# pathwaycom/pathway

Measured on AMD Instinct MI355X. Metric: events/sec (whole node) on WordCount stream + p50 RAG query latency at fixed QPS, higher is better.
Workload: dtype int64/string-dict; 1 GPU; model=wordcount: stream -> groupby(word).count -> output deltas, global_batch=4000000, seq_len=1, parallelism=dp1 (shard exchange: RCCL all-to-all), vocab=50000, ingest=bytes, emitted_delta_rows=126750000, dict_misses=0

## Files before the change

pathway_amd/ops/__init__.py:

```python

from __future__ import annotations

import contextlib
import ctypes
import os
from typing import Sequence

import torch

_THIS = os.path.dirname(os.path.abspath(__file__))
_LIB_PATH = os.path.join(_THIS, "libpwhip.so")

_lib = None
_load_error: Exception | None = None


def _try_load():
    global _lib, _load_error
    if _lib is not None:
        return _lib
    try:
        if not os.path.exists(_LIB_PATH):
            from pathway_amd.ops import build as _build

            _build.build(verbose=False)
        _lib = ctypes.CDLL(_LIB_PATH)
        _lib.pw_hash128_words.restype = ctypes.c_int
        _lib.pw_value_hash.restype = ctypes.c_int
        _lib.pw_varlen_hash.restype = ctypes.c_int
        _lib.pw_run_starts.restype = ctypes.c_int
    except Exception as e:
        _load_error = e
        _lib = None
    return _lib


def lib_available() -> bool:
    return _try_load() is not None


def require_lib():
    lib = _try_load()
    if lib is None:
        raise RuntimeError(
            f"pathway_amd native HIP library missing on a GPU host: {_load_error}"
        )
    return lib


def _stream_ptr() -> ctypes.c_void_p:
    return ctypes.c_void_p(torch.cuda.current_stream().cuda_stream)


def hash128_words_gpu(words: Sequence[torch.Tensor]) -> tuple[torch.Tensor, torch.Tensor]:
    lib = require_lib()
    n = words[0].shape[0]
    lo = torch.empty(n, dtype=torch.int64, device=words[0].device)
    hi = torch.empty(n, dtype=torch.int64, device=words[0].device)
    arr = (ctypes.c_void_p * len(words))(
        *[ctypes.c_void_p(w.contiguous().data_ptr()) for w in words]
    )
    rc = lib.pw_hash128_words(
        arr,
        ctypes.c_int(len(words)),
        ctypes.c_int64(n),
        ctypes.c_void_p(lo.data_ptr()),
        ctypes.c_void_p(hi.data_ptr()),
        _stream_ptr(),
    )
    if rc != 0:
        raise RuntimeError(f"pw_hash128_words failed: hip error {rc}")
    return lo, hi


def value_hash_gpu(payload: torch.Tensor, tag: int) -> tuple[torch.Tensor, torch.Tensor]:
    lib = require_lib()
    payload = payload.contiguous()
    n = payload.shape[0]
    lo = torch.empty(n, dtype=torch.int64, device=payload.device)
    hi = torch.empty(n, dtype=torch.int64, device=payload.device)
    rc = lib.pw_value_hash(
        ctypes.c_void_p(payload.data_ptr()),
        ctypes.c_uint64(tag),
        ctypes.c_int64(n),
        ctypes.c_void_p(lo.data_ptr()),
        ctypes.c_void_p(hi.data_ptr()),
        _stream_ptr(),
    )
    if rc != 0:
        raise RuntimeError(f"pw_value_hash failed: hip error {rc}")
    return lo, hi


def varlen_hash_gpu(
    bytes_t: torch.Tensor, offsets: torch.Tensor, tag: int
) -> tuple[torch.Tensor, torch.Tensor]:
    lib = require_lib()
    n = offsets.shape[0] - 1
    lo = torch.empty(n, dtype=torch.int64, device=bytes_t.device)
    hi = torch.empty(n, dtype=torch.int64, device=bytes_t.device)
    rc = lib.pw_varlen_hash(
        ctypes.c_void_p(bytes_t.contiguous().data_ptr()),
        ctypes.c_void_p(offsets.contiguous().data_ptr()),
        ctypes.c_uint64(tag),
        ctypes.c_int64(n),
        ctypes.c_void_p(lo.data_ptr()),
        ctypes.c_void_p(hi.data_ptr()),
        _stream_ptr(),
    )
    if rc != 0:
        raise RuntimeError(f"pw_varlen_hash failed: hip error {rc}")
    return lo, hi


def run_starts_gpu(words: Sequence[torch.Tensor]) -> torch.Tensor:
    lib = require_lib()
    n = words[0].shape[0]
    starts = torch.empty(n, dtype=torch.bool, device=words[0].device)
    arr = (ctypes.c_void_p * len(words))(
        *[ctypes.c_void_p(w.contiguous().data_ptr()) for w in words]
    )
    rc = lib.pw_run_starts(
        arr,
        ctypes.c_int(len(words)),
        ctypes.c_int64(n),
        ctypes.c_void_p(starts.data_ptr()),
        _stream_ptr(),
    )
    if rc != 0:
        raise RuntimeError(f"pw_run_starts failed: hip error {rc}")
    return starts


def host_hash128_bytes(data: bytes) -> tuple[int, int]:
    lib = require_lib()
    lo = ctypes.c_uint64()
    hi = ctypes.c_uint64()
    lib.pw_host_hash128_bytes(data, ctypes.c_int64(len(data)), ctypes.byref(lo), ctypes.byref(hi))
    return lo.value, hi.value


def _ptr_arr(tensors):
    return (ctypes.c_void_p * len(tensors))(
        *[ctypes.c_void_p(t.data_ptr()) for t in tensors]
    )


def searchsorted_gpu(
    sorted_words: Sequence[torch.Tensor],
    query_words: Sequence[torch.Tensor],
    side: str = "left",
) -> torch.Tensor:
    lib = require_lib()
    m = sorted_words[0].shape[0]
    nq = query_words[0].shape[0]
    out = torch.empty(nq, dtype=torch.int64, device=query_words[0].device)
    s = [t.contiguous() for t in sorted_words]
    q = [t.contiguous() for t in query_words]
    rc = lib.pw_searchsorted(
        _ptr_arr(s),
        _ptr_arr(q),
        ctypes.c_int(len(s)),
        ctypes.c_int64(m),
        ctypes.c_int64(nq),
        ctypes.c_int(1 if side == "right" else 0),
        ctypes.c_void_p(out.data_ptr()),
        _stream_ptr(),
    )
    if rc != 0:
        raise RuntimeError(f"pw_searchsorted failed: hip error {rc}")
    return out


def lookup_gpu(
    sorted_words: Sequence[torch.Tensor], query_words: Sequence[torch.Tensor]
) -> tuple[torch.Tensor, torch.Tensor]:
    lib = require_lib()
    m = sorted_words[0].shape[0]
    nq = query_words[0].shape[0]
    pos = torch.empty(nq, dtype=torch.int64, device=query_words[0].device)
    found = torch.empty(nq, dtype=torch.bool, device=query_words[0].device)
    s = [t.contiguous() for t in sorted_words]
    q = [t.contiguous() for t in query_words]
    rc = lib.pw_lookup(
        _ptr_arr(s),
        _ptr_arr(q),
        ctypes.c_int(len(s)),
        ctypes.c_int64(m),
        ctypes.c_int64(nq),
        ctypes.c_void_p(pos.data_ptr()),
        ctypes.c_void_p(found.data_ptr()),
        _stream_ptr(),
    )
    if rc != 0:
        raise RuntimeError(f"pw_lookup failed: hip error {rc}")
    return pos, found


def key_range_gpu(
    sorted_words: Sequence[torch.Tensor], query_words: Sequence[torch.Tensor]
) -> tuple[torch.Tensor, torch.Tensor]:
    lib = require_lib()
    m = sorted_words[0].shape[0]
    nq = query_words[0].shape[0]
    lo = torch.empty(nq, dtype=torch.int64, device=query_words[0].device)
    hi = torch.empty(nq, dtype=torch.int64, device=query_words[0].device)
    s = [t.contiguous() for t in sorted_words]
    q = [t.contiguous() for t in query_words]
    rc = lib.pw_key_range(
        _ptr_arr(s),
        _ptr_arr(q),
        ctypes.c_int(len(s)),
        ctypes.c_int64(m),
        ctypes.c_int64(nq),
        ctypes.c_void_p(lo.data_ptr()),
        ctypes.c_void_p(hi.data_ptr()),
        _stream_ptr(),
    )
    if rc != 0:
        raise RuntimeError(f"pw_key_range failed: hip error {rc}")
    return lo, hi


SEG_FIRST = 0
SEG_MIN = 1
SEG_MAX = 2
SEG_SELECT_LONG = 4096
SEG_DISTINCT_CAPACITY = 4096
SEG_DISTINCT_MAX_PASSES = 64

multiset_path_counts = {"select": 0, "distinct": 0, "host": 0, "torch": 0}


def _check_ranges(lo: torch.Tensor, hi: torch.Tensor, weights: torch.Tensor):
    for name, t in (("lo", lo), ("hi", hi), ("weights", weights)):
        if t.dtype != torch.int64 or t.dim() != 1 or not t.is_contiguous():
            raise ValueError(f"{name} must be a contiguous 1-D int64 tensor")
        if not t.is_cuda or t.device != weights.device:
            raise ValueError(f"{name} must be on the weights' GPU")
    if lo.shape[0] != hi.shape[0]:
        raise ValueError("lo and hi differ in length")


def seg_select_gpu(
    lo: torch.Tensor,
    hi: torch.Tensor,
    weights: torch.Tensor,
    key: torch.Tensor | None,
    mode: int,
    long_rows: int | None = None,
) -> torch.Tensor:
    lib = require_lib()
    _check_ranges(lo, hi, weights)
    m = weights.shape[0]
    if mode == SEG_FIRST:
        if key is not None:
            raise ValueError("SEG_FIRST reads no key")
        kind, kptr = 0, None
    elif mode in (SEG_MIN, SEG_MAX):
        if key is None:
            raise ValueError("SEG_MIN / SEG_MAX need a key column")
        if key.dtype == torch.int64:
            kind = 1
        elif key.dtype == torch.float64:
            kind = 2
        else:
            raise ValueError(f"key must be int64 or float64, not {key.dtype}")
        if key.shape != (m,) or not key.is_contiguous() or key.device != weights.device:
            raise ValueError("key must be a contiguous 1-D column of the store")
        kptr = key.data_ptr()
    else:
        raise ValueError(f"unknown mode {mode}")
    long_rows = SEG_SELECT_LONG if long_rows is None else int(long_rows)
    if long_rows < 64:
        raise ValueError("long_rows must be at least 64")
    nq = lo.shape[0]
    sel = torch.empty(nq, dtype=torch.int64, device=weights.device)
    rc = lib.pw_seg_select(
        ctypes.c_void_p(lo.data_ptr()),
        ctypes.c_void_p(hi.data_ptr()),
        ctypes.c_int64(nq),
        ctypes.c_void_p(weights.data_ptr()),
        ctypes.c_void_p(kptr),
        ctypes.c_int(kind),
        ctypes.c_int64(m),
        ctypes.c_int(mode),
        ctypes.c_int64(long_rows),
        ctypes.c_void_p(sel.data_ptr()),
        _stream_ptr(),
    )
    if rc != 0:
        raise RuntimeError(f"pw_seg_select failed: error {rc}")
    return sel


def seg_distinct_gpu(
    lo: torch.Tensor,
    hi: torch.Tensor,
    weights: torch.Tensor,
    values: torch.Tensor,
    table_capacity: int | None = None,
) -> tuple[torch.Tensor, torch.Tensor, torch.Tensor]:
    lib = require_lib()
    _check_ranges(lo, hi, weights)
    m = weights.shape[0]
    if (
        values.dtype != torch.int64
        or values.shape != (m,)
        or not values.is_contiguous()
        or values.device != weights.device
    ):
        raise ValueError("values must be a contiguous 1-D int64 column of the store")
    cap = SEG_DISTINCT_CAPACITY if table_capacity is None else int(table_capacity)
    if cap < 64 or cap > 8192 or cap & (cap - 1):
        raise ValueError("table_capacity must be a power of two in [64, 8192]")
    nq = lo.shape[0]
    dev = weights.device
    count = torch.empty(nq, dtype=torch.int64, device=dev)
    first = torch.empty(nq, dtype=torch.int64, device=dev)
    status = torch.empty(nq, dtype=torch.int32, device=dev)
    rc = lib.pw_seg_distinct(
        ctypes.c_void_p(lo.data_ptr()),
        ctypes.c_void_p(hi.data_ptr()),
        ctypes.c_int64(nq),
        ctypes.c_void_p(weights.data_ptr()),
        ctypes.c_void_p(values.data_ptr()),
        ctypes.c_int64(m),
        ctypes.c_int64(cap),
        ctypes.c_int64(int(GC_BUCKET_MAX_LOAD * cap)),
        ctypes.c_int64(GC_BUCKET_MAX_PROBE),
        ctypes.c_void_p(count.data_ptr()),
        ctypes.c_void_p(first.data_ptr()),
        ctypes.c_void_p(status.data_ptr()),
        _stream_ptr(),
    )
    if rc != 0:
        raise RuntimeError(f"pw_seg_distinct failed: error {rc}")
    return count, first, status


def pool_hash_gpu(
    codes: torch.Tensor,
    pool_lo: torch.Tensor,
    pool_hi: torch.Tensor,
    none_lo: int,
    none_hi: int,
) -> tuple[torch.Tensor, torch.Tensor]:
    lib = require_lib()
    n = codes.shape[0]
    lo = torch.empty(n, dtype=torch.int64, device=codes.device)
    hi = torch.empty(n, dtype=torch.int64, device=codes.device)
    rc = lib.pw_pool_hash(
        ctypes.c_void_p(codes.contiguous().data_ptr()),
        ctypes.c_void_p(pool_lo.contiguous().data_ptr()),
        ctypes.c_void_p(pool_hi.contiguous().data_ptr()),
        ctypes.c_uint64(none_lo & ((1 << 64) - 1)),
        ctypes.c_uint64(none_hi & ((1 << 64) - 1)),
        ctypes.c_int64(n),
        ctypes.c_void_p(lo.data_ptr()),
        ctypes.c_void_p(hi.data_ptr()),
        _stream_ptr(),
    )
    if rc != 0:
        raise RuntimeError(f"pw_pool_hash failed: hip error {rc}")
    return lo, hi


def varlen_hash_se_gpu(
    bytes_t: torch.Tensor,
    starts: torch.Tensor,
    ends: torch.Tensor,
    tag: int,
) -> tuple[torch.Tensor, torch.Tensor]:
    lib = require_lib()
    n = starts.shape[0]
    lo = torch.empty(n, dtype=torch.int64, device=bytes_t.device)
    hi = torch.empty(n, dtype=torch.int64, device=bytes_t.device)
    rc = lib.pw_varlen_hash_se(
        ctypes.c_void_p(bytes_t.contiguous().data_ptr()),
        ctypes.c_void_p(starts.contiguous().data_ptr()),
        ctypes.c_void_p(ends.contiguous().data_ptr()),
        ctypes.c_uint64(tag),
        ctypes.c_int64(n),
        ctypes.c_void_p(lo.data_ptr()),
        ctypes.c_void_p(hi.data_ptr()),
        _stream_ptr(),
    )
    if rc != 0:
        raise RuntimeError(f"pw_varlen_hash_se failed: hip error {rc}")
    return lo, hi


def hash_agg_gpu(
    k0: torch.Tensor,
    k1: torch.Tensor,
    contribs: Sequence[torch.Tensor],
    expected_uniques: int | None = None,
) -> tuple[torch.Tensor, torch.Tensor, list, torch.Tensor] | None:
    lib = require_lib()
    n = k0.shape[0]
    dev = k0.device
    nacc = len(contribs)
    est = n if expected_uniques is None else min(max(expected_uniques, 512), n)
    cap = 1 << max(10, (2 * est - 1).bit_length())
    out_cap = min(n, cap)
    tk0 = torch.empty(cap, dtype=torch.int64, device=dev)
    tk1 = torch.zeros(cap, dtype=torch.int64, device=dev)
    rep = torch.zeros(cap, dtype=torch.int64, device=dev)
    taccs = [torch.zeros(cap, dtype=torch.int64, device=dev) for _ in range(nacc)]
    counter = torch.zeros(2, dtype=torch.int32, device=dev)
    out_k0 = torch.empty(out_cap, dtype=torch.int64, device=dev)
    out_k1 = torch.empty(out_cap, dtype=torch.int64, device=dev)
    out_rep = torch.empty(out_cap, dtype=torch.int64, device=dev)
    out_accs = [
        torch.empty(out_cap, dtype=torch.int64, device=dev) for _ in range(nacc)
    ]
    carr = (ctypes.c_void_p * max(nacc, 1))(
        *[ctypes.c_void_p(c.contiguous().data_ptr()) for c in contribs]
    )
    tarr = (ctypes.c_void_p * max(nacc, 1))(
        *[ctypes.c_void_p(c.data_ptr()) for c in taccs]
    )
    oarr = (ctypes.c_void_p * max(nacc, 1))(
        *[ctypes.c_void_p(c.data_ptr()) for c in out_accs]
    )
    rc = lib.pw_hash_agg(
        ctypes.c_void_p(k0.contiguous().data_ptr()),
        ctypes.c_void_p(k1.contiguous().data_ptr()),
        carr,
        ctypes.c_int(nacc),
        ctypes.c_int64(n),
        ctypes.c_void_p(tk0.data_ptr()),
        ctypes.c_void_p(tk1.data_ptr()),
        tarr,
        ctypes.c_void_p(rep.data_ptr()),
        ctypes.c_int64(cap),
        ctypes.c_void_p(counter.data_ptr()),
        ctypes.c_void_p(out_k0.data_ptr()),
        ctypes.c_void_p(out_k1.data_ptr()),
        oarr,
        ctypes.c_void_p(out_rep.data_ptr()),
        ctypes.c_void_p(counter.data_ptr() + 4),
        _stream_ptr(),
    )
    if rc != 0:
        raise RuntimeError(f"pw_hash_agg failed: hip error {rc}")
    m, overflowed = (int(x) for x in counter.tolist())
    if overflowed:
        return None
    return (
        out_k0.narrow(0, 0, m),
        out_k1.narrow(0, 0, m),
        [a.narrow(0, 0, m) for a in out_accs],
        out_rep.narrow(0, 0, m),
    )


def seg_reduce_words_gpu(
    words: Sequence[torch.Tensor], contribs: Sequence[torch.Tensor]
) -> tuple[list, torch.Tensor, list]:
    lib = require_lib()
    n = words[0].shape[0]
    dev = words[0].device
    nw = len(words)
    nacc = len(contribs)
    words = [w.contiguous() for w in words]
    nblocks = (n + 255) // 256
    block_counts = torch.empty(nblocks, dtype=torch.int32, device=dev)
    warr = (ctypes.c_void_p * nw)(
        *[ctypes.c_void_p(w.data_ptr()) for w in words]
    )
    rc = lib.pw_seg_reduce_count(
        warr,
        ctypes.c_int(nw),
        ctypes.c_int64(n),
        ctypes.c_void_p(block_counts.data_ptr()),
        ctypes.c_int64(nblocks),
        _stream_ptr(),
    )
    if rc != 0:
        raise RuntimeError(f"pw_seg_reduce_count failed: hip error {rc}")
    csum = torch.cumsum(block_counts.to(torch.int64), 0)
    nseg = int(csum[-1].item())
    bases = torch.cat(
        [torch.zeros(1, dtype=torch.int64, device=dev), csum[:-1]]
    )
    out_words = [torch.empty(nseg, dtype=torch.int64, device=dev) for _ in range(nw)]
    out_first = torch.empty(nseg, dtype=torch.int64, device=dev)
    out_accs = [torch.zeros(nseg, dtype=torch.int64, device=dev) for _ in range(nacc)]
    carr = (ctypes.c_void_p * max(nacc, 1))(
        *[ctypes.c_void_p(c.contiguous().data_ptr()) for c in contribs]
    )
    oarr = (ctypes.c_void_p * max(nacc, 1))(
        *[ctypes.c_void_p(c.data_ptr()) for c in out_accs]
    )
    owarr = (ctypes.c_void_p * nw)(
        *[ctypes.c_void_p(w.data_ptr()) for w in out_words]
    )
    rc = lib.pw_seg_reduce_emit(
        warr,
        ctypes.c_int(nw),
        carr,
        ctypes.c_int(nacc),
        ctypes.c_int64(n),
        ctypes.c_void_p(bases.data_ptr()),
        owarr,
        ctypes.c_void_p(out_first.data_ptr()),
        oarr,
        ctypes.c_int64(nblocks),
        _stream_ptr(),
    )
    if rc != 0:
        raise RuntimeError(f"pw_seg_reduce_emit failed: hip error {rc}")
    return out_words, out_first, out_accs


def seg_reduce_gpu(
    k0: torch.Tensor, k1: torch.Tensor, contribs: Sequence[torch.Tensor]
) -> tuple[torch.Tensor, torch.Tensor, torch.Tensor, list]:
    out_words, out_first, out_accs = seg_reduce_words_gpu([k0, k1], contribs)
    return out_words[0], out_words[1], out_first, out_accs


_gc_temp_bytes: dict[int, int] = {}
_gc_temp_bytes_prefix: dict[int, int] = {}

_PW_GC_FULL_SORT = bool(os.environ.get("PW_GC_FULL_SORT"))

class _GcPathCounts(dict):

    bucket = 0

    def __getitem__(self, key):
        return self.bucket if key == "bucket" else dict.__getitem__(self, key)

    def __setitem__(self, key, value):
        if key == "bucket":
            self.bucket = value
        else:
            dict.__setitem__(self, key, value)


gc_path_counts = _GcPathCounts({"prefix": 0, "fallback": 0, "full": 0})

_PW_NO_GC_PARTITION = bool(os.environ.get("PW_NO_GC_PARTITION"))
_PW_GC_PART_DIRECT = bool(os.environ.get("PW_GC_PART_DIRECT"))
gc_bucket_layout_counts = {"partition": 0, "gather": 0}
GC_PART_TILE = 8192
GC_PART_MAX_BITS = 8

_gc_bucket_scope = False


@contextlib.contextmanager
def gc_bucket_scope(on: bool):
    global _gc_bucket_scope
    old, _gc_bucket_scope = _gc_bucket_scope, bool(on)
    try:
        yield
    finally:
        _gc_bucket_scope = old

gc_last_dirty_runs = 0

GC_BUCKET_MAX_LOAD = 0.5
GC_BUCKET_BITS = 8
GC_BUCKET_ROWS_FACTOR = 4
GC_BUCKET_MAX_PROBE = 128
GC_BUCKET_ROWS_FLOOR = 65536

_gc_bucket_caps: dict[int, int] = {}


def gc_bucket_capacity_limit(nacc: int) -> int:
    cap = _gc_bucket_caps.get(nacc)
    if cap is None:
        fn = require_lib().pw_gc_bucket_max_capacity
        fn.restype = ctypes.c_int64
        cap = int(fn(ctypes.c_int(nacc)))
        if cap < 2:
            raise RuntimeError("pw_gc_bucket_max_capacity failed")
        _gc_bucket_caps[nacc] = cap
    return cap


def gc_bucket_capacity(nacc: int) -> int:
    return min(gc_bucket_capacity_limit(nacc), 2048)


def gc_bucket_key_budget(nacc: int, bucket_bits: int = GC_BUCKET_BITS,
                         table_capacity: int | None = None) -> int:
    cap = table_capacity or gc_bucket_capacity(nacc)
    return (1 << bucket_bits) * int(GC_BUCKET_MAX_LOAD * cap)


def _gc_temp(lib, n: int, prefix: bool, dev) -> tuple[torch.Tensor, int]:
    cache = _gc_temp_bytes_prefix if prefix else _gc_temp_bytes
    tbytes = cache.get(n)
    if tbytes is None:
        fn = lib.pw_gc_temp_bytes_prefix if prefix else lib.pw_gc_temp_bytes
        fn.restype = ctypes.c_int64
        tbytes = int(fn(ctypes.c_int64(n)))
        if tbytes <= 0:
            raise RuntimeError("pw_gc_temp_bytes failed")
        cache[n] = tbytes
    return torch.empty(tbytes, dtype=torch.uint8, device=dev), tbytes


def _group_combine_two_sorts(keys_n2, contribs):
    k0, k1 = keys_n2[:, 0], keys_n2[:, 1]
    perm = torch.argsort(k1, stable=True)
    perm = perm.index_select(0, torch.argsort(k0.index_select(0, perm), stable=True))
    uk0, uk1, first_sorted, accs = seg_reduce_gpu(
        k0.index_select(0, perm),
        k1.index_select(0, perm),
        [c.index_select(0, perm) for c in contribs],
    )
    return uk0, uk1, perm.index_select(0, first_sorted), accs


def _gc_part_hist_entries(lib, n: int, bucket_bits: int) -> int:
    fn = lib.pw_gc_part_hist_entries
    fn.restype = ctypes.c_int64
    entries = int(fn(ctypes.c_int64(n), ctypes.c_int(bucket_bits)))
    if entries <= 0:
        raise RuntimeError("pw_gc_part_hist_entries failed")
    tile = lib.pw_gc_part_tile
    tile.restype = ctypes.c_int64
    assert int(tile()) == GC_PART_TILE
    return entries


def _gc_aligned_keys(keys_n2: torch.Tensor) -> torch.Tensor:
    return keys_n2.clone() if keys_n2.data_ptr() % 16 else keys_n2


def gc_partition_gpu(
    keys_n2: torch.Tensor, contribs: Sequence[torch.Tensor], bucket_bits: int
) -> tuple[torch.Tensor, torch.Tensor, torch.Tensor, list]:
    lib = require_lib()
    n = keys_n2.shape[0]
    dev = keys_n2.device
    nacc = len(contribs)
    assert keys_n2.dim() == 2 and keys_n2.shape[1] == 2
    assert keys_n2.dtype == torch.int64
    assert 2 <= n < 2**32 - 1 and nacc <= 8 and 1 <= bucket_bits <= 8
    if keys_n2.stride() != (2, 1):
        keys_n2 = keys_n2.contiguous()
    keys_n2 = _gc_aligned_keys(keys_n2)
    contribs = [c.contiguous() for c in contribs]
    assert all(c.dtype == torch.int64 and c.shape == (n,) for c in contribs)
    nb = 1 << bucket_bits
    hist = _gc_part_hist_entries(lib, n, bucket_bits)
    part64 = torch.empty((2 + nacc, n), dtype=torch.int64, device=dev)
    scratch32 = torch.empty(hist + n + nb + 1, dtype=torch.int32, device=dev)
    ctl = torch.empty(2, dtype=torch.int64, device=dev)
    carr = (ctypes.c_void_p * max(nacc, 1))(
        *[ctypes.c_void_p(c.data_ptr()) for c in contribs]
    )
    parr = (ctypes.c_void_p * max(nacc, 1))(
        *[ctypes.c_void_p(part64[2 + a].data_ptr()) for a in range(nacc)]
    )
    rc = lib.pw_gc_partition(
        ctypes.c_void_p(keys_n2.data_ptr()),
        ctypes.c_int64(n),
        ctypes.c_int(bucket_bits),
        carr,
        ctypes.c_int(nacc),
        ctypes.c_void_p(scratch32.data_ptr()),
        ctypes.c_void_p(part64.data_ptr()),
        ctypes.c_void_p(scratch32[hist:].data_ptr()),
        parr,
        ctypes.c_void_p(scratch32[hist + n :].data_ptr()),
        ctypes.c_void_p(ctl.data_ptr()),
        ctypes.c_int(int(_PW_GC_PART_DIRECT)),
        _stream_ptr(),
    )
    if rc != 0:
        raise RuntimeError(f"pw_gc_partition failed: hip error {rc}")
    u32 = lambda t: t.to(torch.int64) & 0xFFFFFFFF
    return (
        u32(scratch32[hist + n :]),
# ... 637 lines not shown
    )
    if rc != 0:
        raise RuntimeError(f"pw_merge_consolidate_emit failed: {rc}")
    return out_words, out_accs, rep


def group_update_gpu(
    a_words: Sequence[torch.Tensor],
    a_accs: Sequence[torch.Tensor],
    b_words: Sequence[torch.Tensor],
    b_accs: Sequence[torch.Tensor],
    out_slots: Sequence[int],
):
    lib = require_lib()
    m = a_words[0].shape[0]
    n = b_words[0].shape[0]
    nacc = len(a_accs)
    assert len(a_words) == 2 and len(b_words) == 2
    assert len(b_accs) == nacc and 1 <= nacc <= 8
    slots = sorted(set(int(s) for s in out_slots))
    assert all(0 <= s < nacc for s in slots)
    mask = 0
    for s in slots:
        mask |= 1 << s
    device = b_words[0].device
    nthreads = max(1, (m + n + 7) // 8)
    counts = torch.empty(nthreads * 4, dtype=torch.int32, device=device)
    bases = torch.empty(nthreads * 3, dtype=torch.int64, device=device)
    totals = torch.empty(3, dtype=torch.int64, device=device)
    wA = [t.contiguous() for t in a_words]
    wB = [t.contiguous() for t in b_words]
    aA = [t.contiguous() for t in a_accs]
    aB = [t.contiguous() for t in b_accs]
    for t in wA + wB + aA + aB:
        assert t.dtype == torch.int64
    rc = lib.pw_group_update_count(
        _ptr_arr(wA),
        _ptr_arr(aA),
        _ptr_arr(wB),
        _ptr_arr(aB),
        ctypes.c_int(nacc),
        ctypes.c_uint(mask),
        ctypes.c_int64(m),
        ctypes.c_int64(n),
        ctypes.c_void_p(counts.data_ptr()),
        ctypes.c_void_p(bases.data_ptr()),
        ctypes.c_void_p(totals.data_ptr()),
        ctypes.c_int64(nthreads),
        _stream_ptr(),
    )
    if rc != 0:
        raise RuntimeError(f"pw_group_update_count failed: {rc}")
    n_keep, n_ret, n_ins = totals.tolist()
    n_out = n_ret + n_ins

    def i64(k):
        return torch.empty(k, dtype=torch.int64, device=device)

    out_words = [i64(n_keep) for _ in range(2)]
    out_accs = [i64(n_keep) for _ in range(nacc)]
    rep = i64(n_keep)
    keys = torch.empty((n_out, 2), dtype=torch.int64, device=device)
    diffs = i64(n_out)
    vals = {s: i64(n_out) for s in slots}
    src = i64(n_out)
    varr = (ctypes.c_void_p * 8)(
        *[ctypes.c_void_p(vals[s].data_ptr() if s in vals else 0) for s in range(8)]
    )
    rc = lib.pw_group_update_emit(
        _ptr_arr(wA),
        _ptr_arr(aA),
        _ptr_arr(wB),
        _ptr_arr(aB),
        ctypes.c_int(nacc),
        ctypes.c_uint(mask),
        ctypes.c_int64(m),
        ctypes.c_int64(n),
        ctypes.c_void_p(bases.data_ptr()),
        ctypes.c_int64(n_ret),
        ctypes.c_int64(nthreads),
        _ptr_arr(out_words),
        _ptr_arr(out_accs),
        ctypes.c_void_p(rep.data_ptr()),
        ctypes.c_void_p(keys.data_ptr()),
        ctypes.c_void_p(diffs.data_ptr()),
        varr,
        ctypes.c_void_p(src.data_ptr()),
        _stream_ptr(),
    )
    if rc != 0:
        raise RuntimeError(f"pw_group_update_emit failed: {rc}")
    return out_words, out_accs, rep, keys, diffs, [vals[s] for s in slots], src


def radix_sort64_gpu(keys: torch.Tensor) -> tuple[torch.Tensor, torch.Tensor]:
    lib = require_lib()
    n = keys.shape[0]
    device = keys.device
    perm = torch.arange(n, dtype=torch.int64, device=device)
    if n <= 1:
        return keys.clone(), perm
    nblocks = max(1, min(1024, (n + (64 * 64) - 1) // (64 * 64)))
    chunk = (n + nblocks * 64 - 1) // (nblocks * 64)
    ka = torch.empty(n, dtype=torch.int64, device=device)
    kb = torch.empty(n, dtype=torch.int64, device=device)
    pa = perm
    pb = torch.empty(n, dtype=torch.int64, device=device)
    rc = lib.pw_radix_flip(
        ctypes.c_void_p(keys.contiguous().data_ptr()),
        ctypes.c_void_p(ka.data_ptr()),
        ctypes.c_int64(n),
        _stream_ptr(),
    )
    if rc != 0:
        raise RuntimeError(f"pw_radix_flip failed: {rc}")
    counts = torch.empty(256 * nblocks, dtype=torch.int32, device=device)
    for p in range(8):
        shift = p * 8
        rc = lib.pw_radix_count(
            ctypes.c_void_p(ka.data_ptr()),
            ctypes.c_int64(n),
            ctypes.c_int(shift),
            ctypes.c_int64(nblocks),
            ctypes.c_int64(chunk),
            ctypes.c_void_p(counts.data_ptr()),
            _stream_ptr(),
        )
        if rc != 0:
            raise RuntimeError(f"pw_radix_count failed: {rc}")
        csum = torch.cumsum(counts.to(torch.int64), 0)
        bases = torch.zeros_like(csum)
        bases[1:] = csum[:-1]
        rc = lib.pw_radix_scatter(
            ctypes.c_void_p(ka.data_ptr()),
            ctypes.c_void_p(pa.data_ptr()),
            ctypes.c_int64(n),
            ctypes.c_int(shift),
            ctypes.c_int64(nblocks),
            ctypes.c_int64(chunk),
            ctypes.c_void_p(bases.data_ptr()),
            ctypes.c_void_p(kb.data_ptr()),
            ctypes.c_void_p(pb.data_ptr()),
            _stream_ptr(),
        )
        if rc != 0:
            raise RuntimeError(f"pw_radix_scatter failed: {rc}")
        ka, kb = kb, ka
        pa, pb = pb, pa
    out = torch.empty(n, dtype=torch.int64, device=device)
    rc = lib.pw_radix_unflip(
        ctypes.c_void_p(ka.data_ptr()),
        ctypes.c_void_p(out.data_ptr()),
        ctypes.c_int64(n),
        _stream_ptr(),
    )
    if rc != 0:
        raise RuntimeError(f"pw_radix_unflip failed: {rc}")
    return out, pa


def scan_positions_gpu(buf: torch.Tensor, target: int) -> torch.Tensor:
    lib = require_lib()
    n = buf.shape[0]
    device = buf.device
    nblocks = max(1, min(2048, (n + 4095) // 4096))
    counts = torch.empty(nblocks, dtype=torch.int64, device=device)
    rc = lib.pw_scan_positions(
        ctypes.c_void_p(buf.contiguous().data_ptr()),
        ctypes.c_int64(n),
        ctypes.c_int(int(target)),
        ctypes.c_void_p(counts.data_ptr()),
        ctypes.c_int64(nblocks),
        _stream_ptr(),
    )
    if rc != 0:
        raise RuntimeError(f"pw_scan_positions failed: {rc}")
    csum = torch.cumsum(counts, 0)
    total = int(csum[-1].item())
    bases = torch.zeros(nblocks, dtype=torch.int64, device=device)
    bases[1:] = csum[:-1]
    out = torch.empty(total, dtype=torch.int64, device=device)
    rc = lib.pw_scan_emit(
        ctypes.c_void_p(buf.contiguous().data_ptr()),
        ctypes.c_int64(n),
        ctypes.c_int(int(target)),
        ctypes.c_void_p(bases.data_ptr()),
        ctypes.c_int64(nblocks),
        ctypes.c_void_p(out.data_ptr()),
        _stream_ptr(),
    )
    if rc != 0:
        raise RuntimeError(f"pw_scan_emit failed: {rc}")
    return out


def sort_repair_gpu(
    k0_sorted: torch.Tensor,
    k1_sorted: torch.Tensor,
    perm: torch.Tensor,
    passes: int = 4,
) -> None:
    lib = require_lib()
    n = k0_sorted.shape[0]
    if n < 2:
        return
    rc = lib.pw_sort_repair(
        ctypes.c_void_p(k0_sorted.data_ptr()),
        ctypes.c_void_p(k1_sorted.data_ptr()),
        ctypes.c_void_p(perm.data_ptr()),
        ctypes.c_int64(n),
        ctypes.c_int(int(passes)),
        _stream_ptr(),
    )
    if rc != 0:
        raise RuntimeError(f"pw_sort_repair failed: hip error {rc}")


def gather_cols_gpu(idx: torch.Tensor, cols: list) -> list:
    lib = require_lib()
    m = idx.shape[0]
    outs: list = [None] * len(cols)
    fused_pos: list[int] = []
    for i, c in enumerate(cols):
        if c.dim() == 1 and c.element_size() == 8 and c.is_contiguous():
            fused_pos.append(i)
        else:
            outs[i] = c[idx] if c.dim() > 1 else c.index_select(0, idx)
    idx = idx.contiguous()
    for start in range(0, len(fused_pos), 8):
        group = fused_pos[start : start + 8]
        srcs = (ctypes.c_void_p * len(group))()
        dsts = (ctypes.c_void_p * len(group))()
        for k, i in enumerate(group):
            c = cols[i]
            out = torch.empty(m, dtype=c.dtype, device=c.device)
            outs[i] = out
            srcs[k] = c.data_ptr()
            dsts[k] = out.data_ptr()
        rc = lib.pw_gather_cols(
            ctypes.c_void_p(idx.data_ptr()),
            ctypes.c_int64(m),
            ctypes.c_int(len(group)),
            srcs,
            dsts,
            _stream_ptr(),
        )
        if rc != 0:
            raise RuntimeError(f"pw_gather_cols failed: {rc}")
    return outs


def intern_error_message(e: int) -> str:
    parts = []
    if e & 1:
        parts.append("probe bound hit (table full)")
    if e & 2:
        parts.append("slot, claimer row or span out of range")
    if e & 4:
        parts.append("dictionary arrays or byte arena too small")
    return "device dictionary intern failed: " + "; ".join(parts or [str(e)])


def gather_spans_gpu(
    buf: torch.Tensor,
    starts: torch.Tensor,
    ends: torch.Tensor,
    first_rows: torch.Tensor,
    n_new: torch.Tensor,
    base: torch.Tensor,
    arena: torch.Tensor,
    cursor: torch.Tensor,
    tok_off: torch.Tensor,
    tok_len: torch.Tensor,
    err: torch.Tensor,
) -> None:
    lib = require_lib()
    nrows = starts.shape[0]
    if nrows == 0:
        return
    for t in (buf, starts, ends, first_rows, arena, tok_off, tok_len):
        assert t.is_contiguous()
    rc = lib.pw_gather_spans(
        ctypes.c_void_p(buf.data_ptr()),
        ctypes.c_int64(buf.shape[0]),
        ctypes.c_void_p(starts.data_ptr()),
        ctypes.c_void_p(ends.data_ptr()),
        ctypes.c_int64(nrows),
        ctypes.c_void_p(first_rows.data_ptr()),
        ctypes.c_void_p(n_new.data_ptr()),
        ctypes.c_void_p(base.data_ptr()),
        ctypes.c_void_p(arena.data_ptr()),
        ctypes.c_int64(arena.shape[0]),
        ctypes.c_void_p(cursor.data_ptr()),
        ctypes.c_void_p(tok_off.data_ptr()),
        ctypes.c_void_p(tok_len.data_ptr()),
        ctypes.c_int64(min(tok_off.shape[0], tok_len.shape[0])),
        ctypes.c_void_p(err.data_ptr()),
        _stream_ptr(),
    )
    if rc != 0:
        raise RuntimeError(f"pw_gather_spans failed: hip error {rc}")


class DeviceHashTable:

    def __init__(self, klo: torch.Tensor, khi: torch.Tensor,
                 vals: torch.Tensor | None = None, reserve: int = 0):
        require_lib()
        m = klo.shape[0]
        device = klo.device
        self.nslots = self.slots_for(max(m, int(reserve)))
        self.err = torch.zeros(1, dtype=torch.int64, device=device)
        self._alloc(device)
        self.insert(klo, khi, vals)

    @staticmethod
    def slots_for(m: int) -> int:
        return 1 << max(4, (2 * m - 1).bit_length()) if m else 16

    def _alloc(self, device) -> None:
        nslots = self.nslots
        self.tab_lo = torch.empty(nslots, dtype=torch.int64, device=device)
        self.tab_hi = torch.empty(nslots, dtype=torch.int64, device=device)
        self.tab_val = torch.full((nslots,), -1, dtype=torch.int64, device=device)

    def insert(self, klo: torch.Tensor, khi: torch.Tensor,
               vals: torch.Tensor | None = None) -> None:
        lib = require_lib()
        m = klo.shape[0]
        if not m:
            return
        klo, khi = klo.contiguous(), khi.contiguous()
        vals = vals.contiguous() if vals is not None else None
        rc = lib.pw_ht_build(
            ctypes.c_void_p(klo.data_ptr()),
            ctypes.c_void_p(khi.data_ptr()),
            ctypes.c_void_p(vals.data_ptr()) if vals is not None else None,
            ctypes.c_int64(m),
            ctypes.c_void_p(self.tab_lo.data_ptr()),
            ctypes.c_void_p(self.tab_hi.data_ptr()),
            ctypes.c_void_p(self.tab_val.data_ptr()),
            ctypes.c_int64(self.nslots),
            _stream_ptr(),
        )
        if rc != 0:
            raise RuntimeError(f"pw_ht_build failed: hip error {rc}")

    def fits(self, size: int) -> bool:
        return 2 * int(size) <= self.nslots

    def rebuild(self, size: int, klo: torch.Tensor, khi: torch.Tensor) -> None:
        self.nslots = self.slots_for(max(int(size), klo.shape[0]))
        self._alloc(klo.device)
        self.insert(klo, khi, None)

    def intern(
        self,
        qlo: torch.Tensor,
        qhi: torch.Tensor,
        base,
        pool_lo: torch.Tensor,
        pool_hi: torch.Tensor,
        front: "DeviceHashTable | None" = None,
    ) -> tuple[torch.Tensor, torch.Tensor, torch.Tensor]:
        lib = require_lib()
        n = qlo.shape[0]
        device = qlo.device
        codes = torch.empty(n, dtype=torch.int64, device=device)
        first_rows = torch.empty(n, dtype=torch.int64, device=device)
        if n == 0:
            return codes, first_rows, torch.zeros(1, dtype=torch.int64, device=device)
        if not torch.is_tensor(base):
            base = torch.tensor([int(base)], dtype=torch.int64, device=device)
        assert base.dtype == torch.int64 and base.is_contiguous()
        assert pool_lo.is_contiguous() and pool_hi.is_contiguous()
        qlo, qhi = qlo.contiguous(), qhi.contiguous()
        nblocks = max(1, min(2048, (n + 4095) // 4096))
        work = torch.empty(nblocks + 1, dtype=torch.int64, device=device)
        pend = torch.empty(n, dtype=torch.uint8, device=device)
        n_new = work[nblocks:]
        rc = lib.pw_ht_intern(
            ctypes.c_void_p(qlo.data_ptr()),
            ctypes.c_void_p(qhi.data_ptr()),
            ctypes.c_int64(n),
            ctypes.c_void_p(self.tab_lo.data_ptr()),
            ctypes.c_void_p(self.tab_hi.data_ptr()),
            ctypes.c_void_p(self.tab_val.data_ptr()),
            ctypes.c_int64(self.nslots),
            ctypes.c_void_p(front.tab_lo.data_ptr() if front else None),
            ctypes.c_void_p(front.tab_hi.data_ptr() if front else None),
            ctypes.c_void_p(front.tab_val.data_ptr() if front else None),
            ctypes.c_int64(front.nslots if front else 0),
            ctypes.c_void_p(base.data_ptr()),
            ctypes.c_void_p(pool_lo.data_ptr()),
            ctypes.c_void_p(pool_hi.data_ptr()),
            ctypes.c_int64(min(pool_lo.shape[0], pool_hi.shape[0])),
            ctypes.c_void_p(codes.data_ptr()),
            ctypes.c_void_p(pend.data_ptr()),
            ctypes.c_void_p(first_rows.data_ptr()),
            ctypes.c_void_p(work.data_ptr()),
            ctypes.c_int64(nblocks),
            ctypes.c_void_p(n_new.data_ptr()),
            ctypes.c_void_p(self.err.data_ptr()),
            _stream_ptr(),
        )
        if rc != 0:
            raise RuntimeError(f"pw_ht_intern failed: hip error {rc}")
        return codes, first_rows, n_new

    def check_error(self) -> None:
        e = int(self.err.item())
        if e:
            raise RuntimeError(intern_error_message(e))

    def probe(self, qlo: torch.Tensor, qhi: torch.Tensor) -> tuple[torch.Tensor, torch.Tensor]:
        lib = require_lib()
        nq = qlo.shape[0]
        out = torch.empty(nq, dtype=torch.int64, device=qlo.device)
        found = torch.empty(nq, dtype=torch.bool, device=qlo.device)
        if nq == 0:
            return out, found
        rc = lib.pw_ht_probe(
            ctypes.c_void_p(qlo.contiguous().data_ptr()),
            ctypes.c_void_p(qhi.contiguous().data_ptr()),
            ctypes.c_int64(nq),
            ctypes.c_void_p(self.tab_lo.data_ptr()),
            ctypes.c_void_p(self.tab_hi.data_ptr()),
            ctypes.c_void_p(self.tab_val.data_ptr()),
            ctypes.c_int64(self.nslots),
            ctypes.c_void_p(out.data_ptr()),
            ctypes.c_void_p(found.data_ptr()),
            _stream_ptr(),
        )
        if rc != 0:
            raise RuntimeError(f"pw_ht_probe failed: hip error {rc}")
        return out, found


def gather_all(idx: torch.Tensor, tensors: list) -> list:
    if tensors and tensors[0].is_cuda and idx.shape[0] > 2048 and lib_available():
        return gather_cols_gpu(idx, list(tensors))
    return [
        t.index_select(0, idx) if t.dim() == 1 else t[idx] for t in tensors
    ]
```

pathway_amd/ops/csrc/hip/pw_kernels.hip:

```cpp
#include <hip/hip_runtime.h>
#include <stdint.h>
#include <stdio.h>

#include <cstring>
#include <rocprim/rocprim.hpp>

#include "../xxhash_common.h"

#define PW_BLOCK 256
#define PW_MAX_GRID 2048

static inline int pw_grid(int64_t n) {
  int64_t g = (n + PW_BLOCK - 1) / PW_BLOCK;
  if (g > PW_MAX_GRID) g = PW_MAX_GRID;
  if (g < 1) g = 1;
  return (int)g;
}


struct WordPtrs {
  const uint64_t* p[20];
};

template <int W>
__global__ void k_hash128_words(WordPtrs ptrs, int64_t n, uint64_t* lo,
                                uint64_t* hi) {
  for (int64_t i = (int64_t)blockIdx.x * blockDim.x + threadIdx.x; i < n;
       i += (int64_t)gridDim.x * blockDim.x) {
    uint64_t w[W];
#pragma unroll
    for (int j = 0; j < W; ++j) w[j] = ptrs.p[j][i];
    lo[i] = pw_xxh64_words<W>(w, PW_SEED_LO);
    hi[i] = pw_xxh64_words<W>(w, PW_SEED_HI);
  }
}

extern "C" int pw_hash128_words(const void** word_ptrs, int nwords, int64_t n,
                                void* lo, void* hi, void* stream) {
  WordPtrs ptrs;
  for (int j = 0; j < nwords && j < 20; ++j)
    ptrs.p[j] = (const uint64_t*)word_ptrs[j];
  hipStream_t s = (hipStream_t)stream;
  dim3 grid(pw_grid(n)), block(PW_BLOCK);
#define CASE(W)                                                        \
  case W:                                                              \
    hipLaunchKernelGGL((k_hash128_words<W>), grid, block, 0, s, ptrs,  \
                       n, (uint64_t*)lo, (uint64_t*)hi);               \
    break;
  switch (nwords) {
    CASE(1) CASE(2) CASE(3) CASE(4) CASE(5) CASE(6) CASE(7) CASE(8)
    CASE(9) CASE(10) CASE(11) CASE(12) CASE(13) CASE(14) CASE(15) CASE(16)
    CASE(17) CASE(18) CASE(19) CASE(20)
    default:
      return -1;
  }
#undef CASE
  return (int)hipGetLastError();
}

__global__ void k_value_hash(const uint64_t* payload, uint64_t tag, int64_t n,
                             uint64_t* lo, uint64_t* hi) {
  for (int64_t i = (int64_t)blockIdx.x * blockDim.x + threadIdx.x; i < n;
       i += (int64_t)gridDim.x * blockDim.x) {
    uint64_t w[2] = {tag, payload[i]};
    lo[i] = pw_xxh64_words<2>(w, PW_SEED_LO);
    hi[i] = pw_xxh64_words<2>(w, PW_SEED_HI);
  }
}

extern "C" int pw_value_hash(const void* payload, uint64_t tag, int64_t n,
                             void* lo, void* hi, void* stream) {
  hipLaunchKernelGGL(k_value_hash, dim3(pw_grid(n)), dim3(PW_BLOCK), 0,
                     (hipStream_t)stream, (const uint64_t*)payload, tag, n,
                     (uint64_t*)lo, (uint64_t*)hi);
  return (int)hipGetLastError();
}

__device__ uint64_t pw_xxh64_long(const uint8_t* data, int64_t n, uint64_t tag,
                                  uint64_t seed);

__global__ void k_varlen_hash(const uint8_t* bytes, const int64_t* offsets,
                              uint64_t tag, int64_t n, uint64_t* lo,
                              uint64_t* hi) {
  for (int64_t i = (int64_t)blockIdx.x * blockDim.x + threadIdx.x; i < n;
       i += (int64_t)gridDim.x * blockDim.x) {
    int64_t a = offsets[i], b = offsets[i + 1];
    uint8_t buf[64];
    int64_t len = b - a;
    if (len <= 56) {
      uint64_t t = tag;
      __builtin_memcpy(buf, &t, 8);
      for (int64_t k = 0; k < len; ++k) buf[8 + k] = bytes[a + k];
      lo[i] = pw_xxh64_bytes(buf, 8 + len, PW_SEED_LO);
      hi[i] = pw_xxh64_bytes(buf, 8 + len, PW_SEED_HI);
    } else {
      lo[i] = pw_xxh64_long(bytes + a, len, tag, PW_SEED_LO);
      hi[i] = pw_xxh64_long(bytes + a, len, tag, PW_SEED_HI);
    }
  }
}

__device__ uint64_t pw_xxh64_long(const uint8_t* data, int64_t n, uint64_t tag,
                                  uint64_t seed) {
  uint64_t v1 = seed + PW_P1 + PW_P2;
  uint64_t v2 = seed + PW_P2;
  uint64_t v3 = seed;
  uint64_t v4 = seed - PW_P1;
  uint64_t a = tag, b, c, d;
  __builtin_memcpy(&b, data, 8);
  __builtin_memcpy(&c, data + 8, 8);
  __builtin_memcpy(&d, data + 16, 8);
  v1 = pw_round(v1, a);
  v2 = pw_round(v2, b);
  v3 = pw_round(v3, c);
  v4 = pw_round(v4, d);
  int64_t i = 24;
  while (i + 32 <= n) {
    __builtin_memcpy(&a, data + i, 8);
    __builtin_memcpy(&b, data + i + 8, 8);
    __builtin_memcpy(&c, data + i + 16, 8);
    __builtin_memcpy(&d, data + i + 24, 8);
    v1 = pw_round(v1, a);
    v2 = pw_round(v2, b);
    v3 = pw_round(v3, c);
    v4 = pw_round(v4, d);
    i += 32;
  }
  uint64_t h = pw_rotl64(v1, 1) + pw_rotl64(v2, 7) + pw_rotl64(v3, 12) +
               pw_rotl64(v4, 18);
  h = pw_merge_round(h, v1);
  h = pw_merge_round(h, v2);
  h = pw_merge_round(h, v3);
  h = pw_merge_round(h, v4);
  h += (uint64_t)(n + 8);
  while (i + 8 <= n) {
    uint64_t k;
    __builtin_memcpy(&k, data + i, 8);
    h ^= pw_round(0, k);
    h = pw_rotl64(h, 27) * PW_P1 + PW_P4;
    i += 8;
  }
  while (i + 4 <= n) {
    uint32_t k;
    __builtin_memcpy(&k, data + i, 4);
    h ^= (uint64_t)k * PW_P1;
    h = pw_rotl64(h, 23) * PW_P2 + PW_P3;
    i += 4;
  }
  while (i < n) {
    h ^= (uint64_t)data[i] * PW_P5;
    h = pw_rotl64(h, 11) * PW_P1;
    i += 1;
  }
  return pw_avalanche(h);
}

extern "C" int pw_varlen_hash(const void* bytes, const void* offsets,
                              uint64_t tag, int64_t n, void* lo, void* hi,
                              void* stream) {
  hipLaunchKernelGGL(k_varlen_hash, dim3(pw_grid(n)), dim3(PW_BLOCK), 0,
                     (hipStream_t)stream, (const uint8_t*)bytes,
                     (const int64_t*)offsets, tag, n, (uint64_t*)lo,
                     (uint64_t*)hi);
  return (int)hipGetLastError();
}


struct Words4 {
  const uint64_t* p[4];
};

__global__ void k_run_starts(Words4 w, int nw, int64_t n, bool* starts) {
  for (int64_t i = (int64_t)blockIdx.x * blockDim.x + threadIdx.x; i < n;
       i += (int64_t)gridDim.x * blockDim.x) {
    bool ne = (i == 0);
    if (i > 0) {
      for (int j = 0; j < nw; ++j) ne |= (w.p[j][i] != w.p[j][i - 1]);
    }
    starts[i] = ne;
  }
}

extern "C" int pw_run_starts(const void** word_ptrs, int nwords, int64_t n,
                             void* starts, void* stream) {
  Words4 w;
  for (int j = 0; j < nwords && j < 4; ++j) w.p[j] = (const uint64_t*)word_ptrs[j];
  hipLaunchKernelGGL(k_run_starts, dim3(pw_grid(n)), dim3(PW_BLOCK), 0,
                     (hipStream_t)stream, w, nwords, n, (bool*)starts);
  return (int)hipGetLastError();
}


extern "C" void pw_host_hash128_bytes(const void* data, int64_t n,
                                      uint64_t* lo, uint64_t* hi) {
  *lo = pw_xxh64_bytes((const uint8_t*)data, n, PW_SEED_LO);
  *hi = pw_xxh64_bytes((const uint8_t*)data, n, PW_SEED_HI);
}

extern "C" void pw_host_varlen_hash(const void* bytes, const int64_t* offsets,
                                    uint64_t tag, int64_t n, uint64_t* lo,
                                    uint64_t* hi) {
  const uint8_t* b = (const uint8_t*)bytes;
  for (int64_t i = 0; i < n; ++i) {
    int64_t a = offsets[i], e = offsets[i + 1];
    int64_t len = e - a;
    uint8_t stackbuf[4096];
    uint8_t* buf = stackbuf;
    if (len + 8 > (int64_t)sizeof(stackbuf)) buf = new uint8_t[len + 8];
    uint64_t t = tag;
    __builtin_memcpy(buf, &t, 8);
    __builtin_memcpy(buf + 8, b + a, len);
    lo[i] = pw_xxh64_bytes(buf, len + 8, PW_SEED_LO);
    hi[i] = pw_xxh64_bytes(buf, len + 8, PW_SEED_HI);
    if (buf != stackbuf) delete[] buf;
  }
}


struct SWords {
  const uint64_t* s[4];
  const uint64_t* q[4];
};

__device__ __forceinline__ int pw_cmp_row(const SWords& w, int nw, int64_t si,
                                          int64_t qi) {
  for (int j = 0; j < nw; ++j) {
    int64_t a = (int64_t)w.s[j][si];
    int64_t b = (int64_t)w.q[j][qi];
    if (a < b) return -1;
    if (a > b) return 1;
  }
  return 0;
}

template <bool RIGHT>
__global__ void k_searchsorted(SWords w, int nw, int64_t m, int64_t nq,
                               int64_t* out) {
  for (int64_t i = (int64_t)blockIdx.x * blockDim.x + threadIdx.x; i < nq;
       i += (int64_t)gridDim.x * blockDim.x) {
    int64_t lo = 0, hi = m;
    while (lo < hi) {
      int64_t mid = (lo + hi) >> 1;
      int c = pw_cmp_row(w, nw, mid, i);
      bool go_right = RIGHT ? (c <= 0) : (c < 0);
      if (go_right)
        lo = mid + 1;
      else
        hi = mid;
    }
    out[i] = lo;
  }
}

extern "C" int pw_searchsorted(const void** sorted_ptrs, const void** query_ptrs,
                               int nwords, int64_t m, int64_t nq, int right,
                               void* out, void* stream) {
  SWords w;
  for (int j = 0; j < nwords && j < 4; ++j) {
    w.s[j] = (const uint64_t*)sorted_ptrs[j];
    w.q[j] = (const uint64_t*)query_ptrs[j];
  }
  dim3 grid(pw_grid(nq)), block(PW_BLOCK);
  if (right)
    hipLaunchKernelGGL((k_searchsorted<true>), grid, block, 0,
                       (hipStream_t)stream, w, nwords, m, nq, (int64_t*)out);
  else
    hipLaunchKernelGGL((k_searchsorted<false>), grid, block, 0,
                       (hipStream_t)stream, w, nwords, m, nq, (int64_t*)out);
  return (int)hipGetLastError();
}

__global__ void k_lookup(SWords w, int nw, int64_t m, int64_t nq, int64_t* pos,
                         bool* found) {
  for (int64_t i = (int64_t)blockIdx.x * blockDim.x + threadIdx.x; i < nq;
       i += (int64_t)gridDim.x * blockDim.x) {
    int64_t lo = 0, hi = m;
    while (lo < hi) {
      int64_t mid = (lo + hi) >> 1;
      if (pw_cmp_row(w, nw, mid, i) < 0)
        lo = mid + 1;
      else
        hi = mid;
    }
    bool f = false;
    int64_t p = lo;
    if (lo < m && pw_cmp_row(w, nw, lo, i) == 0) f = true;
    if (p >= m) p = m > 0 ? m - 1 : 0;
    pos[i] = p;
    found[i] = f;
  }
}

extern "C" int pw_lookup(const void** sorted_ptrs, const void** query_ptrs,
                         int nwords, int64_t m, int64_t nq, void* pos,
                         void* found, void* stream) {
  SWords w;
  for (int j = 0; j < nwords && j < 4; ++j) {
    w.s[j] = (const uint64_t*)sorted_ptrs[j];
    w.q[j] = (const uint64_t*)query_ptrs[j];
  }
  hipLaunchKernelGGL(k_lookup, dim3(pw_grid(nq)), dim3(PW_BLOCK), 0,
                     (hipStream_t)stream, w, nwords, m, nq, (int64_t*)pos,
                     (bool*)found);
  return (int)hipGetLastError();
}

__global__ void k_key_range(SWords w, int nw, int64_t m, int64_t nq,
                            int64_t* lo_out, int64_t* hi_out) {
  for (int64_t i = (int64_t)blockIdx.x * blockDim.x + threadIdx.x; i < nq;
       i += (int64_t)gridDim.x * blockDim.x) {
    int64_t lo = 0, hi = m;
    while (lo < hi) {
      int64_t mid = (lo + hi) >> 1;
      if (pw_cmp_row(w, nw, mid, i) < 0)
        lo = mid + 1;
      else
        hi = mid;
    }
    int64_t left = lo;
    lo = left;
    hi = m;
    while (lo < hi) {
      int64_t mid = (lo + hi) >> 1;
      if (pw_cmp_row(w, nw, mid, i) <= 0)
        lo = mid + 1;
      else
        hi = mid;
    }
    lo_out[i] = left;
    hi_out[i] = lo;
  }
}

extern "C" int pw_key_range(const void** sorted_ptrs, const void** query_ptrs,
                            int nwords, int64_t m, int64_t nq, void* lo,
                            void* hi, void* stream) {
  SWords w;
  for (int j = 0; j < nwords && j < 4; ++j) {
    w.s[j] = (const uint64_t*)sorted_ptrs[j];
    w.q[j] = (const uint64_t*)query_ptrs[j];
  }
  hipLaunchKernelGGL(k_key_range, dim3(pw_grid(nq)), dim3(PW_BLOCK), 0,
                     (hipStream_t)stream, w, nwords, m, nq, (int64_t*)lo,
                     (int64_t*)hi);
  return (int)hipGetLastError();
}


__global__ void k_pool_hash(const int64_t* codes, const uint64_t* pool_lo,
                            const uint64_t* pool_hi, uint64_t none_lo,
                            uint64_t none_hi, int64_t n, uint64_t* lo,
                            uint64_t* hi) {
  for (int64_t i = (int64_t)blockIdx.x * blockDim.x + threadIdx.x; i < n;
       i += (int64_t)gridDim.x * blockDim.x) {
    int64_t c = codes[i];
    if (c >= 0) {
      lo[i] = pool_lo[c];
      hi[i] = pool_hi[c];
    } else {
      lo[i] = none_lo;
      hi[i] = none_hi;
    }
  }
}

extern "C" int pw_pool_hash(const void* codes, const void* pool_lo,
                            const void* pool_hi, uint64_t none_lo,
                            uint64_t none_hi, int64_t n, void* lo, void* hi,
                            void* stream) {
  hipLaunchKernelGGL(k_pool_hash, dim3(pw_grid(n)), dim3(PW_BLOCK), 0,
                     (hipStream_t)stream, (const int64_t*)codes,
                     (const uint64_t*)pool_lo, (const uint64_t*)pool_hi,
                     none_lo, none_hi, n, (uint64_t*)lo, (uint64_t*)hi);
  return (int)hipGetLastError();
}

__global__ void k_varlen_hash_se(const uint8_t* bytes, const int64_t* starts,
                                 const int64_t* ends, uint64_t tag, int64_t n,
                                 uint64_t* lo, uint64_t* hi) {
  for (int64_t i = (int64_t)blockIdx.x * blockDim.x + threadIdx.x; i < n;
       i += (int64_t)gridDim.x * blockDim.x) {
    int64_t a = starts[i], b = ends[i];
    uint8_t buf[64];
    int64_t len = b - a;
    if (len <= 56) {
      uint64_t t = tag;
      __builtin_memcpy(buf, &t, 8);
      for (int64_t k = 0; k < len; ++k) buf[8 + k] = bytes[a + k];
      lo[i] = pw_xxh64_bytes(buf, 8 + len, PW_SEED_LO);
      hi[i] = pw_xxh64_bytes(buf, 8 + len, PW_SEED_HI);
    } else {
      lo[i] = pw_xxh64_long(bytes + a, len, tag, PW_SEED_LO);
      hi[i] = pw_xxh64_long(bytes + a, len, tag, PW_SEED_HI);
    }
  }
}

extern "C" int pw_varlen_hash_se(const void* bytes, const void* starts,
                                 const void* ends, uint64_t tag, int64_t n,
                                 void* lo, void* hi, void* stream) {
  hipLaunchKernelGGL(k_varlen_hash_se, dim3(pw_grid(n)), dim3(PW_BLOCK), 0,
                     (hipStream_t)stream, (const uint8_t*)bytes,
                     (const int64_t*)starts, (const int64_t*)ends, tag, n,
                     (uint64_t*)lo, (uint64_t*)hi);
  return (int)hipGetLastError();
}


#define PW_HA_EMPTY 0x8000000000000000ULL

struct AccPtrs {
  const long long* p[8];
};
struct AccPtrsMut {
  long long* p[8];
};

__global__ void k_hash_agg(const long long* k0, const long long* k1,
                           AccPtrs contribs, int nacc, int64_t n,
                           unsigned long long* tk0, long long* tk1,
                           AccPtrsMut taccs, long long* rep, uint64_t mask,
                           unsigned int* overflow) {
  for (int64_t i = (int64_t)blockIdx.x * blockDim.x + threadIdx.x; i < n;
       i += (int64_t)gridDim.x * blockDim.x) {
    unsigned long long key0 = (unsigned long long)k0[i];
    long long key1 = k1[i];
    uint64_t slot = ((uint64_t)key0) & mask;
    for (uint64_t tries = 0; tries < 512 && tries <= mask; ++tries) {
      unsigned long long cur = tk0[slot];
      if (cur == PW_HA_EMPTY)
        cur = atomicCAS(&tk0[slot], PW_HA_EMPTY, key0);
      if (cur == PW_HA_EMPTY) {
        tk1[slot] = key1;
        rep[slot] = (long long)i;
        __threadfence();
      } else if (cur != key0) {
        slot = (slot + 1) & mask;
        continue;
      } else if (tk1[slot] != key1) {
        slot = (slot + 1) & mask;
        continue;
      }
      for (int a = 0; a < nacc; ++a)
        atomicAdd((unsigned long long*)&taccs.p[a][slot],
                  (unsigned long long)contribs.p[a][i]);
      goto next_row;
    }
    atomicOr(overflow, 1u);
  next_row:;
  }
}

__global__ void k_hash_agg_init(unsigned long long* tk0, uint64_t cap) {
  for (uint64_t i = (uint64_t)blockIdx.x * blockDim.x + threadIdx.x; i < cap;
       i += (uint64_t)gridDim.x * blockDim.x)
    tk0[i] = PW_HA_EMPTY;
}

__global__ void k_hash_agg_collect(const unsigned long long* tk0,
                                   const long long* tk1, AccPtrs taccs,
                                   const long long* rep, int nacc,
                                   uint64_t cap, unsigned int* counter,
                                   long long* out_k0, long long* out_k1,
                                   AccPtrsMut out_accs, long long* out_rep) {
  for (uint64_t i = (uint64_t)blockIdx.x * blockDim.x + threadIdx.x; i < cap;
       i += (uint64_t)gridDim.x * blockDim.x) {
    unsigned long long k = tk0[i];
    if (k == PW_HA_EMPTY) continue;
    unsigned int idx = atomicAdd(counter, 1u);
    out_k0[idx] = (long long)k;
    out_k1[idx] = tk1[i];
    out_rep[idx] = rep[i];
    for (int a = 0; a < nacc; ++a) out_accs.p[a][idx] = taccs.p[a][i];
  }
}

extern "C" int pw_hash_agg(const void* k0, const void* k1,
                           const void** contrib_ptrs, int nacc, int64_t n,
                           void* tk0, void* tk1, void** tacc_ptrs, void* rep,
                           int64_t capacity, void* counter, void* out_k0,
                           void* out_k1, void** out_acc_ptrs, void* out_rep,
                           void* overflow, void* stream) {
  if (nacc > 8) return 1;
  hipStream_t s = (hipStream_t)stream;
  AccPtrs cp;
  AccPtrsMut tp, op;
  for (int a = 0; a < nacc; ++a) {
    cp.p[a] = (const long long*)contrib_ptrs[a];
    tp.p[a] = (long long*)tacc_ptrs[a];
    op.p[a] = (long long*)out_acc_ptrs[a];
  }
  AccPtrs tpc;
  for (int a = 0; a < nacc; ++a) tpc.p[a] = tp.p[a];
  uint64_t mask = (uint64_t)capacity - 1;
  dim3 block(PW_BLOCK);
  hipLaunchKernelGGL(k_hash_agg_init, dim3(pw_grid(capacity)), block, 0, s,
                     (unsigned long long*)tk0, (uint64_t)capacity);
  hipLaunchKernelGGL(k_hash_agg, dim3(pw_grid(n)), block, 0, s,
                     (const long long*)k0, (const long long*)k1, cp, nacc, n,
                     (unsigned long long*)tk0, (long long*)tk1, tp,
                     (long long*)rep, mask, (unsigned int*)overflow);
  hipLaunchKernelGGL(k_hash_agg_collect, dim3(pw_grid(capacity)), block, 0, s,
                     (const unsigned long long*)tk0, (const long long*)tk1,
                     tpc, (long long*)rep, nacc, (uint64_t)capacity,
                     (unsigned int*)counter, (long long*)out_k0,
                     (long long*)out_k1, op, (long long*)out_rep);
  return (int)hipGetLastError();
}


struct SegWords {
  const int64_t* p[8];
};

__global__ void k_segred_count(SegWords w, int nw, int64_t n,
                               int* block_counts) {
  int64_t i = (int64_t)blockIdx.x * blockDim.x + threadIdx.x;
  int flag = 0;
  if (i < n) {
    if (i == 0) flag = 1;
    else {
      for (int j = 0; j < nw; ++j)
        if (w.p[j][i] != w.p[j][i - 1]) { flag = 1; break; }
    }
  }
  __shared__ int cnt[PW_BLOCK / 64];
  int wavecnt = __popcll(__ballot(flag));
  if ((threadIdx.x & 63) == 0) cnt[threadIdx.x >> 6] = wavecnt;
  __syncthreads();
  if (threadIdx.x == 0) {
    int total = 0;
    for (int j = 0; j < PW_BLOCK / 64; ++j) total += cnt[j];
    block_counts[blockIdx.x] = total;
  }
}

__global__ void k_segred_emit(SegWords w, int nw, AccPtrs contribs, int nacc,
                              int64_t n, const long long* block_bases,
                              AccPtrsMut out_words, long long* out_first,
                              AccPtrsMut out_accs) {
  int64_t i = (int64_t)blockIdx.x * blockDim.x + threadIdx.x;
  int lane = threadIdx.x & 63;
  int flag = 0;
  if (i < n) {
    if (i == 0) flag = 1;
    else {
      for (int j = 0; j < nw; ++j)
        if (w.p[j][i] != w.p[j][i - 1]) { flag = 1; break; }
    }
  }
  uint64_t ball = __ballot(flag);
  int wave = threadIdx.x >> 6;
  __shared__ int wave_tot[PW_BLOCK / 64];
  if (lane == 0) wave_tot[wave] = __popcll(ball);
  __syncthreads();
  int wave_base = 0;
  for (int j = 0; j < wave; ++j) wave_base += wave_tot[j];
  uint64_t below = ball & ((lane == 0) ? 0ULL : ((1ULL << lane) - 1));
  int local_excl = wave_base + __popcll(below);
  long long base = block_bases[blockIdx.x];
  long long sid = base + local_excl + flag - 1;
  if (i < n && flag) {
    for (int j = 0; j < nw; ++j) out_words.p[j][sid] = (long long)w.p[j][i];
    out_first[sid] = i;
  }
  long long s = (i < n) ? sid : -1;
  for (int a = 0; a < nacc; ++a) {
    long long v = (i < n) ? contribs.p[a][i] : 0;
#pragma unroll
    for (int off = 1; off < 64; off <<= 1) {
      long long vv = __shfl_up(v, off, 64);
      long long ss = __shfl_up(s, off, 64);
      if (lane >= off && ss == s) v += vv;
    }
    long long nxt = __shfl_down(s, 1, 64);
    bool tail = (lane == 63) || (nxt != s);
    if (s >= 0 && tail)
      atomicAdd((unsigned long long*)&out_accs.p[a][s],
                (unsigned long long)v);
  }
}

extern "C" int pw_seg_reduce_count(const void** word_ptrs, int nw, int64_t n,
                                   void* block_counts, int64_t nblocks,
                                   void* stream) {
  if (nw > 8) return 1;
  SegWords w;
  for (int j = 0; j < nw; ++j) w.p[j] = (const int64_t*)word_ptrs[j];
  hipStream_t s = (hipStream_t)stream;
  hipLaunchKernelGGL(k_segred_count, dim3((uint32_t)nblocks), dim3(PW_BLOCK),
                     0, s, w, nw, n, (int*)block_counts);
  return (int)hipGetLastError();
}

extern "C" int pw_seg_reduce_emit(const void** word_ptrs, int nw,
                                  const void** contrib_ptrs, int nacc,
                                  int64_t n, const void* block_bases,
                                  void** out_word_ptrs, void* out_first,
                                  void** out_acc_ptrs, int64_t nblocks,
                                  void* stream) {
  if (nacc > 8 || nw > 8) return 1;
  SegWords w;
  for (int j = 0; j < nw; ++j) w.p[j] = (const int64_t*)word_ptrs[j];
  AccPtrs cp;
  AccPtrsMut op, ow;
  for (int a = 0; a < nacc; ++a) {
    cp.p[a] = (const long long*)contrib_ptrs[a];
    op.p[a] = (long long*)out_acc_ptrs[a];
  }
  for (int j = 0; j < nw; ++j) ow.p[j] = (long long*)out_word_ptrs[j];
  hipStream_t s = (hipStream_t)stream;
  hipLaunchKernelGGL(k_segred_emit, dim3((uint32_t)nblocks), dim3(PW_BLOCK),
                     0, s, w, nw, cp, nacc, n, (const long long*)block_bases,
                     ow, (long long*)out_first, op);
  return (int)hipGetLastError();
}


#define PW_PART_MAX_DEST 64

__global__ void k_partition_count(const int64_t* dest, int64_t n,
                                  int64_t chunk, int world,
                                  long long* block_hist) {
  __shared__ int hist[PW_PART_MAX_DEST];
  for (int d = threadIdx.x; d < world; d += blockDim.x) hist[d] = 0;
  __syncthreads();
  int64_t start = (int64_t)blockIdx.x * chunk;
  int64_t end = min(start + chunk, n);
  for (int64_t i = start + threadIdx.x; i < end; i += blockDim.x)
    atomicAdd(&hist[(int)dest[i]], 1);
  __syncthreads();
  for (int d = threadIdx.x; d < world; d += blockDim.x)
    block_hist[(int64_t)blockIdx.x * world + d] = hist[d];
}

__global__ void k_partition_scan(long long* block_hist, int64_t nblocks,
                                 int world, long long* counts) {
  if (threadIdx.x == 0) {
    long long run = 0;
    for (int d = 0; d < world; ++d) {
      long long dtotal = 0;
      for (int64_t b = 0; b < nblocks; ++b) {
        long long c = block_hist[b * world + d];
        block_hist[b * world + d] = run;
        run += c;
        dtotal += c;
      }
      counts[d] = dtotal;
    }
  }
}

__global__ void k_partition_scatter(const int64_t* dest, int64_t n,
                                    int64_t chunk, int world,
                                    const long long* block_bases,
                                    int64_t* perm) {
  __shared__ unsigned int offs[PW_PART_MAX_DEST];
  for (int d = threadIdx.x; d < world; d += blockDim.x) offs[d] = 0;
  __syncthreads();
  int64_t start = (int64_t)blockIdx.x * chunk;
  int64_t end = min(start + chunk, n);
  const long long* base = block_bases + (int64_t)blockIdx.x * world;
  for (int64_t i = start + threadIdx.x; i < end; i += blockDim.x) {
    int d = (int)dest[i];
    unsigned int p = atomicAdd(&offs[d], 1u);
    perm[base[d] + p] = i;
  }
}

extern "C" int pw_partition(const void* dest, int64_t n, int world,
                            void* perm, void* counts, void* scratch,
                            int64_t nblocks, void* stream) {
  if (world > PW_PART_MAX_DEST) return 2;
  hipStream_t s = (hipStream_t)stream;
  int64_t chunk = (n + nblocks - 1) / nblocks;
  if (chunk < 1) chunk = 1;
  hipLaunchKernelGGL(k_partition_count, dim3((uint32_t)nblocks),
                     dim3(PW_BLOCK), 0, s, (const int64_t*)dest, n, chunk,
                     world, (long long*)scratch);
  hipLaunchKernelGGL(k_partition_scan, dim3(1), dim3(1), 0, s,
                     (long long*)scratch, nblocks, world,
                     (long long*)counts);
  hipLaunchKernelGGL(k_partition_scatter, dim3((uint32_t)nblocks),
                     dim3(PW_BLOCK), 0, s, (const int64_t*)dest, n, chunk,
                     world, (const long long*)scratch, (int64_t*)perm);
  return (int)hipGetLastError();
}


typedef __attribute__((ext_vector_type(8))) __bf16 pw_frag8;
typedef __attribute__((ext_vector_type(4))) float pw_frag4f;

#define PW_GEMM_BM 128
#define PW_GEMM_BN 128
#define PW_GEMM_BK 64

__device__ __forceinline__ float pw_gelu(float x) {
  return 0.5f * x * (1.0f + erff(x * 0.70710678118654752f));
}

template <int NBUF>
__global__ __launch_bounds__(256) void k_gemm_bf16(
    const __bf16* __restrict__ A, const __bf16* __restrict__ Bt,
    const float* __restrict__ bias, __bf16* __restrict__ C, int64_t M,
    int64_t N, int64_t K, int act, int nbm) {
// ... 719 lines not shown
                     (int4*)thread_counts, nthreads);
  hipLaunchKernelGGL(k_gu_scan, dim3(1), dim3(PW_GU_SCAN_THREADS), 0, s,
                     (const int4*)thread_counts, nthreads, (int64_t*)bases,
                     (int64_t*)totals);
  return (int)hipGetLastError();
}

extern "C" int pw_group_update_emit(
    const void** wordsA, const void** accA, const void** wordsB,
    const void** accB, int nacc, unsigned out_slots, int64_t m, int64_t n,
    const void* bases, int64_t n_ret, int64_t nthreads, void** out_words,
    void** out_accs, void* rep, void* out_keys, void* out_diffs,
    void** out_vals, void* src, void* stream) {
  if (nacc > 8 || nacc < 1 || nthreads < 1) return 2;
  McAcc A{}, B{};
  McWords WA{}, WB{};
  gu_args(wordsA, accA, wordsB, accB, nacc, &WA, &A, &WB, &B);
  GuOut O{};
  for (int k = 0; k < 2; ++k) O.words[k] = (int64_t*)out_words[k];
  for (int c = 0; c < nacc; ++c) {
    O.accs[c] = (long long*)out_accs[c];
    if ((out_slots >> c) & 1u) O.vals[c] = (long long*)out_vals[c];
  }
  O.rep = (int64_t*)rep;
  O.keys = (int64_t*)out_keys;
  O.diffs = (int64_t*)out_diffs;
  O.src = (int64_t*)src;
  hipStream_t s = (hipStream_t)stream;
  int64_t blocks = (nthreads + PW_BLOCK - 1) / PW_BLOCK;
  hipLaunchKernelGGL(k_gu_emit, dim3((uint32_t)blocks), dim3(PW_BLOCK), 0, s,
                     WA, A, WB, B, nacc, out_slots, m, n,
                     (const int64_t*)bases, n_ret, nthreads, O);
  return (int)hipGetLastError();
}


#define PW_RS_THREADS 64
#define PW_RS_DIGITS 256

__global__ __launch_bounds__(PW_RS_THREADS) void k_rs_flip(
    const int64_t* in, uint64_t* out, int64_t n, int dir) {
  for (int64_t i = (int64_t)blockIdx.x * blockDim.x + threadIdx.x; i < n;
       i += (int64_t)gridDim.x * blockDim.x)
    out[i] = (uint64_t)in[i] ^ 0x8000000000000000ull;
}

__global__ __launch_bounds__(PW_RS_THREADS) void k_rs_count(
    const uint64_t* keys, int64_t n, int shift, int64_t chunk,
    int* block_digit_counts ,
    int64_t nblocks) {
  __shared__ int cnt[PW_RS_THREADS][PW_RS_DIGITS];
  int lane = threadIdx.x;
  for (int d = 0; d < PW_RS_DIGITS; ++d) cnt[lane][d] = 0;
  int64_t start = ((int64_t)blockIdx.x * PW_RS_THREADS + lane) * chunk;
  int64_t end = min(start + chunk, n);
  for (int64_t i = start; i < end; ++i) {
    int d = (int)((keys[i] >> shift) & 0xFF);
    ++cnt[lane][d];
  }
  __syncthreads();
  for (int d = lane; d < PW_RS_DIGITS; d += PW_RS_THREADS) {
    int s = 0;
    for (int t = 0; t < PW_RS_THREADS; ++t) s += cnt[t][d];
    block_digit_counts[(int64_t)d * nblocks + blockIdx.x] = s;
  }
}

__global__ __launch_bounds__(PW_RS_THREADS) void k_rs_scatter(
    const uint64_t* keys, const int64_t* payload, int64_t n, int shift,
    int64_t chunk, const long long* bases ,
    int64_t nblocks, uint64_t* out_keys, int64_t* out_payload) {
  __shared__ long long lane_base[PW_RS_THREADS][PW_RS_DIGITS];
  int lane = threadIdx.x;
  for (int d = 0; d < PW_RS_DIGITS; ++d) lane_base[lane][d] = 0;
  int64_t start = ((int64_t)blockIdx.x * PW_RS_THREADS + lane) * chunk;
  int64_t end = min(start + chunk, n);
  for (int64_t i = start; i < end; ++i) {
    int d = (int)((keys[i] >> shift) & 0xFF);
    ++lane_base[lane][d];
  }
  __syncthreads();
  for (int d = lane; d < PW_RS_DIGITS; d += PW_RS_THREADS) {
    long long run = bases[(int64_t)d * nblocks + blockIdx.x];
    for (int t = 0; t < PW_RS_THREADS; ++t) {
      long long c = lane_base[t][d];
      lane_base[t][d] = run;
      run += c;
    }
  }
  __syncthreads();
  for (int64_t i = start; i < end; ++i) {
    int d = (int)((keys[i] >> shift) & 0xFF);
    long long p = lane_base[lane][d]++;
    out_keys[p] = keys[i];
    out_payload[p] = payload[i];
  }
}

__global__ __launch_bounds__(PW_RS_THREADS) void k_rs_unflip(
    const uint64_t* in, int64_t* out, int64_t n) {
  for (int64_t i = (int64_t)blockIdx.x * blockDim.x + threadIdx.x; i < n;
       i += (int64_t)gridDim.x * blockDim.x)
    out[i] = (int64_t)(in[i] ^ 0x8000000000000000ull);
}

extern "C" int pw_radix_flip(const void* in, void* out, int64_t n,
                             void* stream) {
  hipStream_t s = (hipStream_t)stream;
  int64_t blocks = min((int64_t)2048, (n + PW_RS_THREADS - 1) / PW_RS_THREADS);
  if (blocks < 1) blocks = 1;
  hipLaunchKernelGGL(k_rs_flip, dim3((uint32_t)blocks), dim3(PW_RS_THREADS),
                     0, s, (const int64_t*)in, (uint64_t*)out, n, 0);
  return (int)hipGetLastError();
}

extern "C" int pw_radix_unflip(const void* in, void* out, int64_t n,
                               void* stream) {
  hipStream_t s = (hipStream_t)stream;
  int64_t blocks = min((int64_t)2048, (n + PW_RS_THREADS - 1) / PW_RS_THREADS);
  if (blocks < 1) blocks = 1;
  hipLaunchKernelGGL(k_rs_unflip, dim3((uint32_t)blocks),
                     dim3(PW_RS_THREADS), 0, s, (const uint64_t*)in,
                     (int64_t*)out, n);
  return (int)hipGetLastError();
}

extern "C" int pw_radix_count(const void* keys, int64_t n, int shift,
                              int64_t nblocks, int64_t chunk, void* counts,
                              void* stream) {
  hipStream_t s = (hipStream_t)stream;
  hipLaunchKernelGGL(k_rs_count, dim3((uint32_t)nblocks),
                     dim3(PW_RS_THREADS), 0, s, (const uint64_t*)keys, n,
                     shift, chunk, (int*)counts, nblocks);
  return (int)hipGetLastError();
}

extern "C" int pw_radix_scatter(const void* keys, const void* payload,
                                int64_t n, int shift, int64_t nblocks,
                                int64_t chunk, const void* bases,
                                void* out_keys, void* out_payload,
                                void* stream) {
  hipStream_t s = (hipStream_t)stream;
  hipLaunchKernelGGL(k_rs_scatter, dim3((uint32_t)nblocks),
                     dim3(PW_RS_THREADS), 0, s, (const uint64_t*)keys,
                     (const int64_t*)payload, n, shift, chunk,
                     (const long long*)bases, nblocks, (uint64_t*)out_keys,
                     (int64_t*)out_payload);
  return (int)hipGetLastError();
}


__device__ __forceinline__ unsigned pw_granule_mask(const uint8_t* buf,
                                                    int64_t g, int64_t end,
                                                    uint8_t t, bool aligned) {
  unsigned m = 0;
  if (aligned && g + 16 <= end) {
    uint4 v = *(const uint4*)(buf + g);
    const uint32_t w[4] = {v.x, v.y, v.z, v.w};
#pragma unroll
    for (int q = 0; q < 4; ++q)
#pragma unroll
      for (int j = 0; j < 4; ++j)
        if (((w[q] >> (8 * j)) & 0xFFu) == t) m |= 1u << (4 * q + j);
  } else {
    for (int j = 0; j < 16 && g + j < end; ++j)
      if (buf[g + j] == t) m |= 1u << j;
  }
  return m;
}

__global__ void k_scan_count(const uint8_t* buf, int64_t n, int target,
                             int64_t chunk, long long* block_counts) {
  __shared__ int cnt;
  if (threadIdx.x == 0) cnt = 0;
  __syncthreads();
  int64_t start = (int64_t)blockIdx.x * chunk;
  int64_t end = min(start + chunk, n);
  const bool aligned = (((size_t)buf & 15) == 0);
  int local = 0;
  for (int64_t tile = start; tile < end; tile += (int64_t)blockDim.x * 16) {
    int64_t g = tile + (int64_t)threadIdx.x * 16;
    if (g < end)
      local += __popc(pw_granule_mask(buf, g, end, (uint8_t)target, aligned));
  }
  atomicAdd(&cnt, local);
  __syncthreads();
  if (threadIdx.x == 0) block_counts[blockIdx.x] = cnt;
}

__global__ void k_scan_emit(const uint8_t* buf, int64_t n, int target,
                            int64_t chunk, const long long* bases,
                            int64_t* out) {
  const int lane = threadIdx.x & 63;
  const int wave = threadIdx.x >> 6;
  __shared__ long long cursor;
  __shared__ int wave_tot[PW_BLOCK / 64];
  if (threadIdx.x == 0) cursor = bases[blockIdx.x];
  __syncthreads();
  int64_t start = (int64_t)blockIdx.x * chunk;
  int64_t end = min(start + chunk, n);
  const bool aligned = (((size_t)buf & 15) == 0);
  for (int64_t tile = start; tile < end; tile += (int64_t)blockDim.x * 16) {
    int64_t g = tile + (int64_t)threadIdx.x * 16;
    unsigned hmask =
        (g < end) ? pw_granule_mask(buf, g, end, (uint8_t)target, aligned) : 0u;
    int hits = __popc(hmask);
    int incl = hits;
#pragma unroll
    for (int off = 1; off < 64; off <<= 1) {
      int v = __shfl_up(incl, off, 64);
      if (lane >= off) incl += v;
    }
    if (lane == 63) wave_tot[wave] = incl;
    __syncthreads();
    int wbase = 0;
    for (int w = 0; w < wave; ++w) wbase += wave_tot[w];
    long long my = cursor + wbase + (incl - hits);
    while (hmask) {
      int j = __ffs(hmask) - 1;
      hmask &= hmask - 1;
      out[my++] = g + j;
    }
    __syncthreads();
    if (threadIdx.x == (int)blockDim.x - 1) cursor += wbase + incl;
    __syncthreads();
  }
}

extern "C" int pw_scan_positions(const void* buf, int64_t n, int target,
                                 void* block_counts, int64_t nblocks,
                                 void* stream) {
  hipStream_t s = (hipStream_t)stream;
  int64_t chunk = ((n + nblocks - 1) / nblocks + 15) & ~(int64_t)15;
  if (chunk < 16) chunk = 16;
  hipLaunchKernelGGL(k_scan_count, dim3((uint32_t)nblocks), dim3(PW_BLOCK),
                     0, s, (const uint8_t*)buf, n, target,
                     chunk, (long long*)block_counts);
  return (int)hipGetLastError();
}

extern "C" int pw_scan_emit(const void* buf, int64_t n, int target,
                            const void* bases, int64_t nblocks, void* out,
                            void* stream) {
  hipStream_t s = (hipStream_t)stream;
  int64_t chunk = ((n + nblocks - 1) / nblocks + 15) & ~(int64_t)15;
  if (chunk < 16) chunk = 16;
  hipLaunchKernelGGL(k_scan_emit, dim3((uint32_t)nblocks), dim3(PW_BLOCK),
                     0, s, (const uint8_t*)buf, n, target, chunk,
                     (const long long*)bases, (int64_t*)out);
  return (int)hipGetLastError();
}


__global__ void k_sort_repair(const long long* __restrict__ k0,
                              long long* k1, long long* perm, int64_t n,
                              int parity) {
  int64_t i = 2 * ((int64_t)blockIdx.x * blockDim.x + threadIdx.x) + parity;
  if (i + 1 >= n) return;
  if (k0[i] != k0[i + 1]) return;
  long long a = k1[i], b = k1[i + 1];
  if (a > b) {
    k1[i] = b;
    k1[i + 1] = a;
    long long p = perm[i];
    perm[i] = perm[i + 1];
    perm[i + 1] = p;
  }
}

extern "C" int pw_sort_repair(const void* k0, void* k1, void* perm,
                              int64_t n, int passes, void* stream) {
  hipStream_t s = (hipStream_t)stream;
  int64_t pairs = n / 2 + 1;
  int64_t nblocks = (pairs + PW_BLOCK - 1) / PW_BLOCK;
  if (nblocks < 1) nblocks = 1;
  for (int p = 0; p < passes; ++p)
    hipLaunchKernelGGL(k_sort_repair, dim3((uint32_t)nblocks), dim3(PW_BLOCK),
                       0, s, (const long long*)k0, (long long*)k1,
                       (long long*)perm, n, p & 1);
  return (int)hipGetLastError();
}


struct PwGather8 {
  const long long* src[8];
  long long* dst[8];
};

__global__ void k_gather_cols(const long long* __restrict__ idx, int64_t m,
                              int ncols, PwGather8 p) {
  int64_t i = (int64_t)blockIdx.x * blockDim.x + threadIdx.x;
  int64_t stride = (int64_t)gridDim.x * blockDim.x;
  for (; i < m; i += stride) {
    long long j = idx[i];
#pragma unroll 8
    for (int c = 0; c < 8; ++c) {
      if (c >= ncols) break;
      p.dst[c][i] = p.src[c][j];
    }
  }
}


__global__ void k_ht_build(const int64_t* __restrict__ klo,
                           const int64_t* __restrict__ khi,
                           const int64_t* __restrict__ vals, int64_t m,
                           int64_t* tab_lo, int64_t* tab_hi,
                           long long* tab_val, int64_t mask) {
  int64_t i = (int64_t)blockIdx.x * blockDim.x + threadIdx.x;
  int64_t stride = (int64_t)gridDim.x * blockDim.x;
  for (; i < m; i += stride) {
    uint64_t slot = (uint64_t)klo[i] & (uint64_t)mask;
    while (atomicCAS((unsigned long long*)&tab_val[slot],
                     (unsigned long long)(long long)-1,
                     (unsigned long long)(long long)(vals ? vals[i] : i)) !=
           (unsigned long long)(long long)-1)
      slot = (slot + 1) & (uint64_t)mask;
    tab_lo[slot] = klo[i];
    tab_hi[slot] = khi[i];
  }
}

__global__ void k_ht_probe(const int64_t* __restrict__ qlo,
                           const int64_t* __restrict__ qhi, int64_t nq,
                           const int64_t* __restrict__ tab_lo,
                           const int64_t* __restrict__ tab_hi,
                           const long long* __restrict__ tab_val,
                           int64_t mask, int64_t* out, bool* found) {
  int64_t i = (int64_t)blockIdx.x * blockDim.x + threadIdx.x;
  int64_t stride = (int64_t)gridDim.x * blockDim.x;
  for (; i < nq; i += stride) {
    int64_t lo = qlo[i], hi = qhi[i];
    uint64_t slot = (uint64_t)lo & (uint64_t)mask;
    int64_t v = -1;
    for (;;) {
      long long tv = tab_val[slot];
      if (tv == -1) break;
      if (tab_lo[slot] == lo && tab_hi[slot] == hi) {
        v = (int64_t)tv;
        break;
      }
      slot = (slot + 1) & (uint64_t)mask;
    }
    out[i] = v;
    found[i] = v != -1;
  }
}

extern "C" int pw_ht_build(const void* klo, const void* khi, const void* vals,
                           int64_t m, void* tab_lo, void* tab_hi,
                           void* tab_val, int64_t nslots, void* stream) {
  hipStream_t s = (hipStream_t)stream;
  int64_t nblocks = (m + PW_BLOCK - 1) / PW_BLOCK;
  if (nblocks > 4096) nblocks = 4096;
  if (nblocks < 1) nblocks = 1;
  hipLaunchKernelGGL(k_ht_build, dim3((uint32_t)nblocks), dim3(PW_BLOCK), 0, s,
                     (const int64_t*)klo, (const int64_t*)khi,
                     (const int64_t*)vals, m, (int64_t*)tab_lo,
                     (int64_t*)tab_hi, (long long*)tab_val, nslots - 1);
  return (int)hipGetLastError();
}

extern "C" int pw_ht_probe(const void* qlo, const void* qhi, int64_t nq,
                           const void* tab_lo, const void* tab_hi,
                           const void* tab_val, int64_t nslots, void* out,
                           void* found, void* stream) {
  hipStream_t s = (hipStream_t)stream;
  int64_t nblocks = (nq + PW_BLOCK - 1) / PW_BLOCK;
  if (nblocks > 4096) nblocks = 4096;
  if (nblocks < 1) nblocks = 1;
  hipLaunchKernelGGL(k_ht_probe, dim3((uint32_t)nblocks), dim3(PW_BLOCK), 0, s,
                     (const int64_t*)qlo, (const int64_t*)qhi, nq,
                     (const int64_t*)tab_lo, (const int64_t*)tab_hi,
                     (const long long*)tab_val, nslots - 1, (int64_t*)out,
                     (bool*)found);
  return (int)hipGetLastError();
}


#define PW_HT_ERR_PROBE 1
#define PW_HT_ERR_STATE 2
#define PW_HT_ERR_CAPACITY 4

__global__ void k_ht_intern_claim(const int64_t* __restrict__ qlo,
                                  const int64_t* __restrict__ qhi, int64_t n,
                                  const int64_t* tab_lo, const int64_t* tab_hi,
                                  long long* tab_val, int64_t nslots,
                                  const int64_t* __restrict__ front_lo,
                                  const int64_t* __restrict__ front_hi,
                                  const long long* __restrict__ front_val,
                                  int64_t front_nslots,
                                  int64_t* __restrict__ codes,
                                  uint8_t* __restrict__ pend, long long* err) {
  const uint64_t mask = (uint64_t)(nslots - 1);
  const uint64_t fmask = (uint64_t)(front_nslots - 1);
  int64_t i = (int64_t)blockIdx.x * blockDim.x + threadIdx.x;
  int64_t stride = (int64_t)gridDim.x * blockDim.x;
  for (; i < n; i += stride) {
    const int64_t lo = qlo[i], hi = qhi[i];
    if (front_nslots) {
      uint64_t fs = (uint64_t)lo & fmask;
      long long fv = -1;
      for (int64_t probes = 0; probes < front_nslots; ++probes) {
        fv = front_val[fs];
        if (fv < 0 || (front_lo[fs] == lo && front_hi[fs] == hi)) break;
        fs = (fs + 1) & fmask;
        fv = -1;
      }
      if (fv >= 0) {
        codes[i] = (int64_t)fv;
        pend[i] = 0;
        continue;
      }
    }
    const long long me = -(long long)(i + 2);
    uint64_t slot = (uint64_t)lo & mask;
    int64_t out = -1;
    uint8_t p = 0;
    int e = PW_HT_ERR_PROBE;
    long long tv = tab_val[slot];
    for (int64_t probes = 0; probes < nslots; ++probes) {
      if (tv == -1) {
        tv = (long long)atomicCAS((unsigned long long*)&tab_val[slot],
                                  (unsigned long long)(long long)-1,
                                  (unsigned long long)me);
        if (tv == -1) {
          out = (int64_t)slot, p = 1, e = 0;
          break;
        }
      }
      if (tv >= 0) {
        if (tab_lo[slot] == lo && tab_hi[slot] == hi) {
          out = (int64_t)tv, e = 0;
          break;
        }
      } else {
        const int64_t r = -(tv + 2);
        if (r < 0 || r >= n) {
          e = PW_HT_ERR_STATE;
          break;
        }
        if (qlo[r] == lo && qhi[r] == hi) {
          if (me > tv)
            __hip_atomic_fetch_max(&tab_val[slot], me, __ATOMIC_RELAXED,
                                   __HIP_MEMORY_SCOPE_AGENT);
          out = (int64_t)slot, p = 1, e = 0;
          break;
        }
      }
      slot = (slot + 1) & mask;
      tv = tab_val[slot];
    }
    if (e) atomicOr((unsigned long long*)err, (unsigned long long)e);
    codes[i] = out;
    pend[i] = p;
  }
}

__global__ void k_ht_intern_count(int64_t n, int64_t chunk,
                                  const int64_t* __restrict__ codes,
                                  uint8_t* pend, const long long* tab_val,
                                  int64_t nslots, long long* block_counts,
                                  long long* err) {
  __shared__ int cnt;
  if (threadIdx.x == 0) cnt = 0;
  __syncthreads();
  int64_t start = (int64_t)blockIdx.x * chunk;
  int64_t end = min(start + chunk, n);
  int local = 0;
  for (int64_t tile = start; tile < end; tile += (int64_t)blockDim.x * 16) {
    int64_t g = tile + (int64_t)threadIdx.x * 16;
    if (g >= end) continue;
    if (g + 16 <= end) {
      uint4 v = *(const uint4*)(pend + g);
      if ((v.x | v.y | v.z | v.w) == 0) continue;
    }
    for (int64_t i = g; i < min(g + 16, end); ++i) {
      if (!pend[i]) continue;
      int64_t slot = codes[i];
      if (slot < 0 || slot >= nslots) {
        atomicOr((unsigned long long*)err, (unsigned long long)PW_HT_ERR_STATE);
        pend[i] = 0;
        continue;
      }
      if (tab_val[slot] == -(long long)(i + 2)) {
        pend[i] = 2;
        ++local;
      }
    }
  }
  if (local) atomicAdd(&cnt, local);
  __syncthreads();
  if (threadIdx.x == 0) block_counts[blockIdx.x] = cnt;
}

__global__ void k_ht_intern_commit(
    const int64_t* __restrict__ qlo, const int64_t* __restrict__ qhi,
    int64_t n, int64_t chunk, int64_t* codes, const uint8_t* __restrict__ pend,
    const long long* __restrict__ block_counts,
    const long long* __restrict__ base_ptr, int64_t* tab_lo, int64_t* tab_hi,
    long long* tab_val, int64_t* pool_lo, int64_t* pool_hi, int64_t pool_cap,
    int64_t* first_row, long long* n_new, long long* err) {
  const int lane = threadIdx.x & 63;
  const int wave = threadIdx.x >> 6;
  __shared__ unsigned long long cursor;
  __shared__ int wave_tot[PW_BLOCK / 64];
  if (threadIdx.x == 0) cursor = 0;
  __syncthreads();
  unsigned long long part = 0;
  for (int j = threadIdx.x; j < (int)blockIdx.x; j += blockDim.x)
    part += (unsigned long long)block_counts[j];
  if (part) atomicAdd(&cursor, part);
  __syncthreads();
  if (blockIdx.x == gridDim.x - 1 && threadIdx.x == 0)
    n_new[0] = (long long)cursor + block_counts[blockIdx.x];
  const long long base = base_ptr[0];
  int64_t start = (int64_t)blockIdx.x * chunk;
  int64_t end = min(start + chunk, n);
  for (int64_t tile = start; tile < end; tile += (int64_t)blockDim.x * 16) {
    int64_t g = tile + (int64_t)threadIdx.x * 16;
    unsigned wmask = 0;
    if (g < end) {
      bool any = true;
      if (g + 16 <= end) {
        uint4 v = *(const uint4*)(pend + g);
        any = (v.x | v.y | v.z | v.w) != 0;
      }
      if (any)
        for (int j = 0; j < 16 && g + j < end; ++j)
          if (pend[g + j] == 2) wmask |= 1u << j;
    }
    int hits = __popc(wmask);
    int incl = hits;
#pragma unroll
    for (int off = 1; off < 64; off <<= 1) {
      int v = __shfl_up(incl, off, 64);
      if (lane >= off) incl += v;
    }
    if (lane == 63) wave_tot[wave] = incl;
    __syncthreads();
    int wbase = 0;
    for (int w = 0; w < wave; ++w) wbase += wave_tot[w];
    long long k = (long long)cursor + wbase + (incl - hits);
    while (wmask) {
      int j = __ffs(wmask) - 1;
      wmask &= wmask - 1;
      const int64_t i = g + j;
      const int64_t slot = codes[i];
      const long long code = base + k;
      if (code < 0 || code >= pool_cap) {
        atomicOr((unsigned long long*)err,
                 (unsigned long long)PW_HT_ERR_CAPACITY);
      } else {
        const int64_t lo = qlo[i], hi = qhi[i];
        tab_lo[slot] = lo;
        tab_hi[slot] = hi;
        pool_lo[code] = lo;
        pool_hi[code] = hi;
        first_row[k] = i;
        tab_val[slot] = code;
        codes[i] = code;
      }
      ++k;
    }
    __syncthreads();
    if (threadIdx.x == (int)blockDim.x - 1) cursor += wbase + incl;
    __syncthreads();
  }
}

__global__ void k_ht_intern_resolve(int64_t n, int64_t chunk, int64_t* codes,
                                    const uint8_t* __restrict__ pend,
                                    const long long* __restrict__ tab_val) {
  int64_t start = (int64_t)blockIdx.x * chunk;
  int64_t end = min(start + chunk, n);
  for (int64_t tile = start; tile < end; tile += (int64_t)blockDim.x * 16) {
    int64_t g = tile + (int64_t)threadIdx.x * 16;
    if (g >= end) continue;
    if (g + 16 <= end) {
      uint4 v = *(const uint4*)(pend + g);
      if ((v.x | v.y | v.z | v.w) == 0) continue;
    }
    for (int64_t i = g; i < min(g + 16, end); ++i) {
      if (pend[i] != 1) continue;
      long long tv = tab_val[codes[i]];
      codes[i] = tv >= 0 ? (int64_t)tv : -1;
    }
  }
}

static inline int64_t pw_intern_chunk(int64_t n, int64_t nblocks) {
  int64_t chunk = ((n + nblocks - 1) / nblocks + 15) & ~(int64_t)15;
  return chunk < 16 ? 16 : chunk;
}

extern "C" int pw_ht_intern(const void* qlo, const void* qhi, int64_t n,
                            void* tab_lo, void* tab_hi, void* tab_val,
                            int64_t nslots, const void* front_lo,
                            const void* front_hi, const void* front_val,
                            int64_t front_nslots, const void* base_ptr,
                            void* pool_lo, void* pool_hi, int64_t pool_cap,
                            void* codes, void* pend, void* first_row,
                            void* block_counts, int64_t nblocks, void* n_new,
                            void* err, void* stream) {
  if (n <= 0 || nblocks < 1 || nblocks > 2048) return -2;
  if (nslots < 1 || (nslots & (nslots - 1))) return -2;
  if (front_nslots < 0 || (front_nslots & (front_nslots - 1))) return -2;
  hipStream_t s = (hipStream_t)stream;
  int64_t cblocks = (n + PW_BLOCK - 1) / PW_BLOCK;
  if (cblocks > 4096) cblocks = 4096;
  int64_t chunk = pw_intern_chunk(n, nblocks);
  hipLaunchKernelGGL(k_ht_intern_claim, dim3((uint32_t)cblocks),
                     dim3(PW_BLOCK), 0, s, (const int64_t*)qlo,
                     (const int64_t*)qhi, n, (const int64_t*)tab_lo,
                     (const int64_t*)tab_hi, (long long*)tab_val, nslots,
                     (const int64_t*)front_lo, (const int64_t*)front_hi,
                     (const long long*)front_val, front_nslots,
                     (int64_t*)codes, (uint8_t*)pend, (long long*)err);
  hipLaunchKernelGGL(k_ht_intern_count, dim3((uint32_t)nblocks),
                     dim3(PW_BLOCK), 0, s, n, chunk, (const int64_t*)codes,
                     (uint8_t*)pend, (const long long*)tab_val, nslots,
                     (long long*)block_counts, (long long*)err);
  hipLaunchKernelGGL(k_ht_intern_commit, dim3((uint32_t)nblocks),
                     dim3(PW_BLOCK), 0, s, (const int64_t*)qlo,
                     (const int64_t*)qhi, n, chunk, (int64_t*)codes,
                     (const uint8_t*)pend, (const long long*)block_counts,
                     (const long long*)base_ptr, (int64_t*)tab_lo,
                     (int64_t*)tab_hi, (long long*)tab_val, (int64_t*)pool_lo,
                     (int64_t*)pool_hi, pool_cap, (int64_t*)first_row,
                     (long long*)n_new, (long long*)err);
  hipLaunchKernelGGL(k_ht_intern_resolve, dim3((uint32_t)nblocks),
                     dim3(PW_BLOCK), 0, s, n, chunk, (int64_t*)codes,
                     (const uint8_t*)pend, (const long long*)tab_val);
  return (int)hipGetLastError();
}

__global__ void k_gather_spans(const uint8_t* __restrict__ buf, int64_t nbuf,
                               const int64_t* __restrict__ starts,
                               const int64_t* __restrict__ ends, int64_t nrows,
                               const int64_t* __restrict__ first_row,
                               const long long* __restrict__ n_new_ptr,
                               const long long* __restrict__ base_ptr,
                               uint8_t* arena, int64_t arena_cap,
                               unsigned long long* cursor, int64_t* tok_off,
                               int64_t* tok_len, int64_t pool_cap,
                               long long* err) {
  const int lane = threadIdx.x & 63;
  long long n_new = n_new_ptr[0];
  if (n_new > nrows) n_new = nrows;
  const long long base = base_ptr[0];
  const int64_t stride = (int64_t)gridDim.x * blockDim.x;
  const int64_t k0 = (int64_t)blockIdx.x * blockDim.x + threadIdx.x;
  for (int64_t k = k0; k - lane < n_new; k += stride) {
    int64_t s = 0, len = 0;
    bool ok = k < n_new && base + k >= 0 && base + k < pool_cap;
    if (ok) {
      int64_t row = first_row[k];
      ok = row >= 0 && row < nrows;
      if (ok) {
        s = starts[row];
        int64_t e = ends[row];
        ok = s >= 0 && e >= s && e <= nbuf;
        len = ok ? e - s : 0;
      }
    }
    if (k < n_new && !ok)
      atomicOr((unsigned long long*)err,
               (unsigned long long)(base + k < pool_cap ? PW_HT_ERR_STATE
                                                        : PW_HT_ERR_CAPACITY));
    long long incl = len;
#pragma unroll
    for (int off = 1; off < 64; off <<= 1) {
      long long v = __shfl_up(incl, off, 64);
      if (lane >= off) incl += v;
    }
    long long total = __shfl(incl, 63, 64);
    unsigned long long wbase = 0;
    if (lane == 0 && total) wbase = atomicAdd(cursor, (unsigned long long)total);
    wbase = __shfl(wbase, 0, 64);
    if (!ok) continue;
    int64_t off = (int64_t)wbase + (incl - len);
    if (off + len > arena_cap) {
      atomicOr((unsigned long long*)err,
               (unsigned long long)PW_HT_ERR_CAPACITY);
      off = 0, len = 0;
    }
    for (int64_t b = 0; b < len; ++b) arena[off + b] = buf[s + b];
    tok_off[base + k] = off;
    tok_len[base + k] = len;
  }
}

extern "C" int pw_gather_spans(const void* buf, int64_t nbuf,
                               const void* starts, const void* ends,
                               int64_t nrows, const void* first_row,
                               const void* n_new_ptr, const void* base_ptr,
                               void* arena, int64_t arena_cap, void* cursor,
                               void* tok_off, void* tok_len, int64_t pool_cap,
                               void* err, void* stream) {
  if (nrows <= 0) return 0;
  hipStream_t s = (hipStream_t)stream;
  hipLaunchKernelGGL(k_gather_spans, dim3(pw_grid(nrows) > 256 ? 256 : pw_grid(nrows)),
                     dim3(PW_BLOCK), 0, s, (const uint8_t*)buf, nbuf,
                     (const int64_t*)starts, (const int64_t*)ends, nrows,
                     (const int64_t*)first_row, (const long long*)n_new_ptr,
                     (const long long*)base_ptr, (uint8_t*)arena, arena_cap,
                     (unsigned long long*)cursor, (int64_t*)tok_off,
                     (int64_t*)tok_len, pool_cap, (long long*)err);
  return (int)hipGetLastError();
}

extern "C" int pw_gather_cols(const void* idx, int64_t m, int ncols,
                              void* const* srcs, void* const* dsts,
                              void* stream) {
  if (ncols < 1 || ncols > 8) return -2;
  hipStream_t s = (hipStream_t)stream;
  PwGather8 p;
  for (int c = 0; c < ncols; ++c) {
    p.src[c] = (const long long*)srcs[c];
    p.dst[c] = (long long*)dsts[c];
  }
  int64_t nblocks = (m + PW_BLOCK - 1) / PW_BLOCK;
  if (nblocks > 4096) nblocks = 4096;
  if (nblocks < 1) nblocks = 1;
  hipLaunchKernelGGL(k_gather_cols, dim3((uint32_t)nblocks), dim3(PW_BLOCK),
                     0, s, (const long long*)idx, m, ncols, p);
  return (int)hipGetLastError();
}


struct GcWord0 {
  const long long* keys;
  __host__ __device__ long long operator()(uint32_t i) const {
    return keys[2 * (size_t)i];
  }
};

using GcKeyIter =
    rocprim::transform_iterator<rocprim::counting_iterator<uint32_t>, GcWord0,
                                long long>;

static hipError_t gc_sort(void* temp, size_t& temp_bytes, const long long* keys,
                          long long* k0_sorted, uint32_t* perm32, int64_t n,
                          hipStream_t s) {
  GcKeyIter kin(rocprim::counting_iterator<uint32_t>(0), GcWord0{keys});
  rocprim::counting_iterator<uint32_t> vin(0);
  return rocprim::radix_sort_pairs(temp, temp_bytes, kin, k0_sorted, vin,
                                   perm32, (size_t)n, 0, 64, s);
}

__global__ void k_gc_gather_k1(const long long* __restrict__ keys,
                               const uint32_t* __restrict__ perm32,
                               long long* __restrict__ k1_sorted, int64_t n,
                               unsigned long long* ctrl) {
  int64_t i = (int64_t)blockIdx.x * blockDim.x + threadIdx.x;
  int64_t stride = (int64_t)gridDim.x * blockDim.x;
  if (i == 0) {
    ctrl[0] = 0;
    ctrl[1] = 0;
  }
  for (; i < n; i += stride) k1_sorted[i] = keys[2 * (size_t)perm32[i] + 1];
}

__global__ void k_gc_sort_repair(const long long* __restrict__ k0,
                                 long long* k1, uint32_t* perm32, int64_t n,
                                 int parity) {
  int64_t i = 2 * ((int64_t)blockIdx.x * blockDim.x + threadIdx.x) + parity;
  if (i + 1 >= n) return;
  if (k0[i] != k0[i + 1]) return;
  long long a = k1[i], b = k1[i + 1];
  if (a > b) {
    k1[i] = b;
    k1[i + 1] = a;
    uint32_t p = perm32[i];
    perm32[i] = perm32[i + 1];
    perm32[i + 1] = p;
  }
}

__global__ void k_gc_emit(const long long* __restrict__ k0,
                          const long long* __restrict__ k1,
                          const uint32_t* __restrict__ perm32,
                          AccPtrs contribs, int nacc, int64_t n,
                          const long long* __restrict__ block_csum,
                          long long* out_k0, long long* out_k1,
                          long long* out_first, AccPtrsMut out_accs) {
  int64_t i = (int64_t)blockIdx.x * blockDim.x + threadIdx.x;
  int lane = threadIdx.x & 63;
  int flag = 0;
  long long a0 = 0, a1 = 0;
  uint32_t row = 0;
  if (i < n) {
    a0 = k0[i];
    a1 = k1[i];
    row = perm32[i];
    flag = (i == 0) || a0 != k0[i - 1] || a1 != k1[i - 1];
  }
  uint64_t ball = __ballot(flag);
  int wave = threadIdx.x >> 6;
  __shared__ int wave_tot[PW_BLOCK / 64];
  if (lane == 0) wave_tot[wave] = __popcll(ball);
  __syncthreads();
  int wave_base = 0;
  for (int j = 0; j < wave; ++j) wave_base += wave_tot[j];
  uint64_t below = ball & ((lane == 0) ? 0ULL : ((1ULL << lane) - 1));
  int local_excl = wave_base + __popcll(below);
  long long base = blockIdx.x ? block_csum[blockIdx.x - 1] : 0;
  long long sid = base + local_excl + flag - 1;
  if (i < n && flag) {
    out_k0[sid] = a0;
    out_k1[sid] = a1;
    out_first[sid] = (long long)row;
  }
  long long s = (i < n) ? sid : -1;
  long long nxt = __shfl_down(s, 1, 64);
  bool tail = (lane == 63) || (nxt != s);
  for (int a = 0; a < nacc; ++a) {
    long long v = (i < n) ? contribs.p[a][row] : 0;
#pragma unroll
    for (int off = 1; off < 64; off <<= 1) {
      long long vv = __shfl_up(v, off, 64);
      long long ss = __shfl_up(s, off, 64);
      if (lane >= off && ss == s) v += vv;
    }
    if (s >= 0 && tail)
      atomicAdd((unsigned long long*)&out_accs.p[a][s],
                (unsigned long long)v);
  }
}

extern "C" int64_t pw_gc_temp_bytes(int64_t n) {
  size_t bytes = 0;
  if (n <= 0 || n >= ((int64_t)1 << 32)) return 0;
  if (gc_sort(nullptr, bytes, nullptr, nullptr, nullptr, n, 0) != hipSuccess)
    return 0;
  return (int64_t)bytes;
}


#define PW_GC_REPAIR_GRID 64
#define PW_GC_MAX_RUN_LIMIT 3072

struct GcPrefix {
  const long long* keys;
  int drop;
  __host__ __device__ uint32_t operator()(uint32_t i) const {
    uint32_t top = (uint32_t)((uint64_t)keys[2 * (size_t)i] >> 32);
    return (top ^ 0x80000000u) >> drop;
  }
};

using GcPrefixIter =
    rocprim::transform_iterator<rocprim::counting_iterator<uint32_t>, GcPrefix,
                                uint32_t>;

static hipError_t gc_sort_prefix(void* temp, size_t& temp_bytes,
                                 const long long* keys, uint32_t* prefix_sorted,
                                 uint32_t* perm32, int64_t n, int prefix_bits,
                                 hipStream_t s) {
  GcPrefixIter kin(rocprim::counting_iterator<uint32_t>(0),
                   GcPrefix{keys, 32 - prefix_bits});
  rocprim::counting_iterator<uint32_t> vin(0);
  return rocprim::radix_sort_pairs(temp, temp_bytes, kin, prefix_sorted, vin,
                                   perm32, (size_t)n, 0u,
                                   (unsigned int)prefix_bits, s);
}

__global__ void k_gc_gather_k01(const long long* __restrict__ keys,
                                const uint32_t* __restrict__ perm32,
                                long long* __restrict__ k0_sorted,
                                long long* __restrict__ k1_sorted, int64_t n,
                                unsigned long long* ctrl) {
  int64_t i = (int64_t)blockIdx.x * blockDim.x + threadIdx.x;
  int64_t stride = (int64_t)gridDim.x * blockDim.x;
  if (i == 0) {
    ctrl[0] = 0;
    ctrl[1] = 0;
  }
  for (; i < n; i += stride) {
    size_t r = 2 * (size_t)perm32[i];
    k0_sorted[i] = keys[r];
    k1_sorted[i] = keys[r + 1];
  }
}

__global__ void k_gc_mark_dirty(const long long* __restrict__ k0,
                                const long long* __restrict__ k1, int64_t n,
                                int shift, uint32_t max_run,
                                uint32_t max_dirty, uint32_t* dirty_list,
                                unsigned long long* ctrl) {
  int64_t i = (int64_t)blockIdx.x * blockDim.x + threadIdx.x;
  if (i < 1 || i >= n) return;
  long long c0 = k0[i], p0 = k0[i - 1];
  uint64_t pref = (uint64_t)c0 >> shift;
  if (((uint64_t)p0 >> shift) != pref) return;
  long long p1 = k1[i - 1];
  if (c0 == p0 && k1[i] == p1) return;
  int64_t j = i - 1;
  uint32_t steps = 0;
  while (j > 0) {
    long long q0 = k0[j - 1];
    if (((uint64_t)q0 >> shift) != pref) break;
    if (q0 != p0 || k1[j - 1] != p1) return;
    --j;
    if (++steps > max_run) {
      ctrl[0] = 1;
      return;
    }
  }
  unsigned long long slot = atomicAdd(&ctrl[1], 1ULL);
  if (slot < max_dirty) dirty_list[slot] = (uint32_t)j;
  else ctrl[0] = 1;
}

__global__ void k_gc_repair_runs(long long* k0, long long* k1,
                                 uint32_t* perm32, int64_t n, int shift,
                                 uint32_t max_run, uint32_t max_dirty,
                                 const uint32_t* __restrict__ dirty_list,
                                 unsigned long long* ctrl) {
  extern __shared__ long long gc_lds[];
  long long* s0 = gc_lds;
  long long* s1 = gc_lds + max_run;
  uint32_t* sp = (uint32_t*)(gc_lds + 2 * (size_t)max_run);
  __shared__ uint32_t run_len;
  unsigned long long listed = ctrl[1];
  uint32_t cnt = listed < max_dirty ? (uint32_t)listed : max_dirty;
  for (uint32_t e = blockIdx.x; e < cnt; e += gridDim.x) {
    int64_t s = dirty_list[e];
    uint64_t pref = (uint64_t)k0[s] >> shift;
    if (threadIdx.x == 0) run_len = max_run + 1;
    __syncthreads();
    for (uint32_t r = 1 + threadIdx.x; r <= max_run; r += blockDim.x) {
      int64_t idx = s + r;
      if (idx >= n || ((uint64_t)k0[idx] >> shift) != pref) {
        atomicMin(&run_len, r);
        break;
// ... 1423 lines not shown
```

pathway_amd/ops/csrc/xxhash_common.h:

```cpp
#pragma once
#include <stdint.h>

#if defined(__HIPCC__)
#define PW_HD __host__ __device__ __forceinline__
#else
#define PW_HD static inline
#endif

#define PW_P1 0x9E3779B185EBCA87ULL
#define PW_P2 0xC2B2AE3D27D4EB4FULL
#define PW_P3 0x165667B19E3779F9ULL
#define PW_P4 0x85EBCA77C2B2AE63ULL
#define PW_P5 0x27D4EB2F165667C5ULL

#define PW_SEED_LO 0ULL
#define PW_SEED_HI 0x9E3779B185EBCA87ULL

PW_HD uint64_t pw_rotl64(uint64_t x, int r) { return (x << r) | (x >> (64 - r)); }

PW_HD uint64_t pw_round(uint64_t acc, uint64_t inp) {
  acc += inp * PW_P2;
  acc = pw_rotl64(acc, 31);
  return acc * PW_P1;
}

PW_HD uint64_t pw_merge_round(uint64_t acc, uint64_t val) {
  val = pw_round(0, val);
  acc ^= val;
  return acc * PW_P1 + PW_P4;
}

PW_HD uint64_t pw_avalanche(uint64_t h) {
  h ^= h >> 33;
  h *= PW_P2;
  h ^= h >> 29;
  h *= PW_P3;
  h ^= h >> 32;
  return h;
}

template <int W>
PW_HD uint64_t pw_xxh64_words(const uint64_t* w, uint64_t seed) {
  const int nbytes = W * 8;
  uint64_t h;
  int i = 0;
  if (nbytes >= 32) {
    uint64_t v1 = seed + PW_P1 + PW_P2;
    uint64_t v2 = seed + PW_P2;
    uint64_t v3 = seed;
    uint64_t v4 = seed - PW_P1;
    while (i + 4 <= W) {
      v1 = pw_round(v1, w[i]);
      v2 = pw_round(v2, w[i + 1]);
      v3 = pw_round(v3, w[i + 2]);
      v4 = pw_round(v4, w[i + 3]);
      i += 4;
    }
    h = pw_rotl64(v1, 1) + pw_rotl64(v2, 7) + pw_rotl64(v3, 12) + pw_rotl64(v4, 18);
    h = pw_merge_round(h, v1);
    h = pw_merge_round(h, v2);
    h = pw_merge_round(h, v3);
    h = pw_merge_round(h, v4);
  } else {
    h = seed + PW_P5;
  }
  h += (uint64_t)nbytes;
  for (; i < W; ++i) {
    h ^= pw_round(0, w[i]);
    h = pw_rotl64(h, 27) * PW_P1 + PW_P4;
  }
  return pw_avalanche(h);
}

PW_HD uint64_t pw_xxh64_bytes(const uint8_t* data, int64_t n, uint64_t seed) {
  int64_t i = 0;
  uint64_t h;
  if (n >= 32) {
    uint64_t v1 = seed + PW_P1 + PW_P2;
    uint64_t v2 = seed + PW_P2;
    uint64_t v3 = seed;
    uint64_t v4 = seed - PW_P1;
    while (i + 32 <= n) {
      uint64_t a, b, c, d;
      __builtin_memcpy(&a, data + i, 8);
      __builtin_memcpy(&b, data + i + 8, 8);
      __builtin_memcpy(&c, data + i + 16, 8);
      __builtin_memcpy(&d, data + i + 24, 8);
      v1 = pw_round(v1, a);
      v2 = pw_round(v2, b);
      v3 = pw_round(v3, c);
      v4 = pw_round(v4, d);
      i += 32;
    }
    h = pw_rotl64(v1, 1) + pw_rotl64(v2, 7) + pw_rotl64(v3, 12) + pw_rotl64(v4, 18);
    h = pw_merge_round(h, v1);
    h = pw_merge_round(h, v2);
    h = pw_merge_round(h, v3);
    h = pw_merge_round(h, v4);
  } else {
    h = seed + PW_P5;
  }
  h += (uint64_t)n;
  while (i + 8 <= n) {
    uint64_t k;
    __builtin_memcpy(&k, data + i, 8);
    h ^= pw_round(0, k);
    h = pw_rotl64(h, 27) * PW_P1 + PW_P4;
    i += 8;
  }
  while (i + 4 <= n) {
    uint32_t k;
    __builtin_memcpy(&k, data + i, 4);
    h ^= (uint64_t)k * PW_P1;
    h = pw_rotl64(h, 23) * PW_P2 + PW_P3;
    i += 4;
  }
  while (i < n) {
    h ^= (uint64_t)data[i] * PW_P5;
    h = pw_rotl64(h, 11) * PW_P1;
    i += 1;
  }
  return pw_avalanche(h);
}
```

Measured before the change: 3.710 billion events/s.

## Interleave hash-table slots and stream tokens through a fused dual-seed xxhash

Replaces the three separate lo/hi/val hash-table arrays with an interleaved 4-word slot layout, so a probe loads the key with one 16-byte access next to its value. Probing now handles two queries per thread to overlap memory latency. Token hashing no longer copies bytes into a per-thread stack buffer. It reads aligned dwords with bounds checks and computes both seeds in a single pass. The table uses more memory per slot, and the boundary-handling read path adds branching.

```diff
diff --git a/pathway_amd/ops/__init__.py b/pathway_amd/ops/__init__.py
--- a/pathway_amd/ops/__init__.py
+++ b/pathway_amd/ops/__init__.py
@@ -99,8 +99,10 @@
     n = offsets.shape[0] - 1
     lo = torch.empty(n, dtype=torch.int64, device=bytes_t.device)
     hi = torch.empty(n, dtype=torch.int64, device=bytes_t.device)
+    bytes_t = bytes_t.contiguous()
     rc = lib.pw_varlen_hash(
-        ctypes.c_void_p(bytes_t.contiguous().data_ptr()),
+        ctypes.c_void_p(bytes_t.data_ptr()),
+        ctypes.c_int64(bytes_t.numel()),
         ctypes.c_void_p(offsets.contiguous().data_ptr()),
         ctypes.c_uint64(tag),
         ctypes.c_int64(n),
@@ -376,8 +378,10 @@
     n = starts.shape[0]
     lo = torch.empty(n, dtype=torch.int64, device=bytes_t.device)
     hi = torch.empty(n, dtype=torch.int64, device=bytes_t.device)
+    bytes_t = bytes_t.contiguous()
     rc = lib.pw_varlen_hash_se(
-        ctypes.c_void_p(bytes_t.contiguous().data_ptr()),
+        ctypes.c_void_p(bytes_t.data_ptr()),
+        ctypes.c_int64(bytes_t.numel()),
         ctypes.c_void_p(starts.contiguous().data_ptr()),
         ctypes.c_void_p(ends.contiguous().data_ptr()),
         ctypes.c_uint64(tag),
@@ -1621,6 +1625,9 @@
         raise RuntimeError(f"pw_gather_spans failed: hip error {rc}")
 
 
+HT_SLOT_WORDS = 4
+
+
 class DeviceHashTable:
 
     def __init__(self, klo: torch.Tensor, khi: torch.Tensor,
@@ -1638,10 +1645,13 @@
         return 1 << max(4, (2 * m - 1).bit_length()) if m else 16
 
     def _alloc(self, device) -> None:
-        nslots = self.nslots
-        self.tab_lo = torch.empty(nslots, dtype=torch.int64, device=device)
-        self.tab_hi = torch.empty(nslots, dtype=torch.int64, device=device)
-        self.tab_val = torch.full((nslots,), -1, dtype=torch.int64, device=device)
+        if require_lib().pw_ht_slot_words() != HT_SLOT_WORDS:
+            raise RuntimeError("libpwhip.so was built for another HT_SLOT_WORDS")
+        self.tab = torch.full((self.nslots, HT_SLOT_WORDS), -1,
+                              dtype=torch.int64, device=device)
+        self.tab_lo = self.tab[:, 0]
+        self.tab_hi = self.tab[:, 1]
+        self.tab_val = self.tab[:, 2]
 
     def insert(self, klo: torch.Tensor, khi: torch.Tensor,
                vals: torch.Tensor | None = None) -> None:
@@ -1656,9 +1666,7 @@
             ctypes.c_void_p(khi.data_ptr()),
             ctypes.c_void_p(vals.data_ptr()) if vals is not None else None,
             ctypes.c_int64(m),
-            ctypes.c_void_p(self.tab_lo.data_ptr()),
-            ctypes.c_void_p(self.tab_hi.data_ptr()),
-            ctypes.c_void_p(self.tab_val.data_ptr()),
+            ctypes.c_void_p(self.tab.data_ptr()),
             ctypes.c_int64(self.nslots),
             _stream_ptr(),
         )
@@ -1702,13 +1710,9 @@
             ctypes.c_void_p(qlo.data_ptr()),
             ctypes.c_void_p(qhi.data_ptr()),
             ctypes.c_int64(n),
-            ctypes.c_void_p(self.tab_lo.data_ptr()),
-            ctypes.c_void_p(self.tab_hi.data_ptr()),
-            ctypes.c_void_p(self.tab_val.data_ptr()),
+            ctypes.c_void_p(self.tab.data_ptr()),
             ctypes.c_int64(self.nslots),
-            ctypes.c_void_p(front.tab_lo.data_ptr() if front else None),
-            ctypes.c_void_p(front.tab_hi.data_ptr() if front else None),
-            ctypes.c_void_p(front.tab_val.data_ptr() if front else None),
+            ctypes.c_void_p(front.tab.data_ptr() if front else None),
             ctypes.c_int64(front.nslots if front else 0),
             ctypes.c_void_p(base.data_ptr()),
             ctypes.c_void_p(pool_lo.data_ptr()),
@@ -1743,9 +1747,7 @@
             ctypes.c_void_p(qlo.contiguous().data_ptr()),
             ctypes.c_void_p(qhi.contiguous().data_ptr()),
             ctypes.c_int64(nq),
-            ctypes.c_void_p(self.tab_lo.data_ptr()),
-            ctypes.c_void_p(self.tab_hi.data_ptr()),
-            ctypes.c_void_p(self.tab_val.data_ptr()),
+            ctypes.c_void_p(self.tab.data_ptr()),
             ctypes.c_int64(self.nslots),
             ctypes.c_void_p(out.data_ptr()),
             ctypes.c_void_p(found.data_ptr()),
diff --git a/pathway_amd/ops/csrc/hip/pw_kernels.hip b/pathway_amd/ops/csrc/hip/pw_kernels.hip
--- a/pathway_amd/ops/csrc/hip/pw_kernels.hip
+++ b/pathway_amd/ops/csrc/hip/pw_kernels.hip
@@ -76,90 +76,24 @@
   return (int)hipGetLastError();
 }
 
-__device__ uint64_t pw_xxh64_long(const uint8_t* data, int64_t n, uint64_t tag,
-                                  uint64_t seed);
-
-__global__ void k_varlen_hash(const uint8_t* bytes, const int64_t* offsets,
-                              uint64_t tag, int64_t n, uint64_t* lo,
-                              uint64_t* hi) {
+__global__ __launch_bounds__(PW_BLOCK) void k_varlen_hash(
+    const uint8_t* __restrict__ bytes, int64_t nbytes,
+    const int64_t* __restrict__ offsets, uint64_t tag, int64_t n,
+    uint64_t* __restrict__ lo, uint64_t* __restrict__ hi) {
   for (int64_t i = (int64_t)blockIdx.x * blockDim.x + threadIdx.x; i < n;
        i += (int64_t)gridDim.x * blockDim.x) {
-    int64_t a = offsets[i], b = offsets[i + 1];
-    uint8_t buf[64];
-    int64_t len = b - a;
-    if (len <= 56) {
-      uint64_t t = tag;
-      __builtin_memcpy(buf, &t, 8);
-      for (int64_t k = 0; k < len; ++k) buf[8 + k] = bytes[a + k];
-      lo[i] = pw_xxh64_bytes(buf, 8 + len, PW_SEED_LO);
-      hi[i] = pw_xxh64_bytes(buf, 8 + len, PW_SEED_HI);
-    } else {
-      lo[i] = pw_xxh64_long(bytes + a, len, tag, PW_SEED_LO);
-      hi[i] = pw_xxh64_long(bytes + a, len, tag, PW_SEED_HI);
-    }
-  }
-}
-
-__device__ uint64_t pw_xxh64_long(const uint8_t* data, int64_t n, uint64_t tag,
-                                  uint64_t seed) {
-  uint64_t v1 = seed + PW_P1 + PW_P2;
-  uint64_t v2 = seed + PW_P2;
-  uint64_t v3 = seed;
-  uint64_t v4 = seed - PW_P1;
-  uint64_t a = tag, b, c, d;
-  __builtin_memcpy(&b, data, 8);
-  __builtin_memcpy(&c, data + 8, 8);
-  __builtin_memcpy(&d, data + 16, 8);
-  v1 = pw_round(v1, a);
-  v2 = pw_round(v2, b);
-  v3 = pw_round(v3, c);
-  v4 = pw_round(v4, d);
-  int64_t i = 24;
-  while (i + 32 <= n) {
-    __builtin_memcpy(&a, data + i, 8);
-    __builtin_memcpy(&b, data + i + 8, 8);
-    __builtin_memcpy(&c, data + i + 16, 8);
-    __builtin_memcpy(&d, data + i + 24, 8);
-    v1 = pw_round(v1, a);
-    v2 = pw_round(v2, b);
-    v3 = pw_round(v3, c);
-    v4 = pw_round(v4, d);
-    i += 32;
-  }
-  uint64_t h = pw_rotl64(v1, 1) + pw_rotl64(v2, 7) + pw_rotl64(v3, 12) +
-               pw_rotl64(v4, 18);
-  h = pw_merge_round(h, v1);
-  h = pw_merge_round(h, v2);
-  h = pw_merge_round(h, v3);
-  h = pw_merge_round(h, v4);
-  h += (uint64_t)(n + 8);
-  while (i + 8 <= n) {
-    uint64_t k;
-    __builtin_memcpy(&k, data + i, 8);
-    h ^= pw_round(0, k);
-    h = pw_rotl64(h, 27) * PW_P1 + PW_P4;
-    i += 8;
-  }
-  while (i + 4 <= n) {
-    uint32_t k;
-    __builtin_memcpy(&k, data + i, 4);
-    h ^= (uint64_t)k * PW_P1;
-    h = pw_rotl64(h, 23) * PW_P2 + PW_P3;
-    i += 4;
-  }
-  while (i < n) {
-    h ^= (uint64_t)data[i] * PW_P5;
-    h = pw_rotl64(h, 11) * PW_P1;
-    i += 1;
-  }
-  return pw_avalanche(h);
-}
-
-extern "C" int pw_varlen_hash(const void* bytes, const void* offsets,
-                              uint64_t tag, int64_t n, void* lo, void* hi,
-                              void* stream) {
+    const int64_t a = offsets[i], b = offsets[i + 1];
+    const PwHash128 h = pw_xxh64_tagged2(bytes, nbytes, a, b - a, tag);
+    lo[i] = h.lo;
+    hi[i] = h.hi;
+  }
+}
+
+extern "C" int pw_varlen_hash(const void* bytes, int64_t nbytes,
+                              const void* offsets, uint64_t tag, int64_t n,
+                              void* lo, void* hi, void* stream) {
   hipLaunchKernelGGL(k_varlen_hash, dim3(pw_grid(n)), dim3(PW_BLOCK), 0,
-                     (hipStream_t)stream, (const uint8_t*)bytes,
+                     (hipStream_t)stream, (const uint8_t*)bytes, nbytes,
                      (const int64_t*)offsets, tag, n, (uint64_t*)lo,
                      (uint64_t*)hi);
   return (int)hipGetLastError();
@@ -201,18 +135,12 @@
                                     uint64_t tag, int64_t n, uint64_t* lo,
                                     uint64_t* hi) {
   const uint8_t* b = (const uint8_t*)bytes;
+  const int64_t nbytes = n > 0 ? offsets[n] : 0;
   for (int64_t i = 0; i < n; ++i) {
-    int64_t a = offsets[i], e = offsets[i + 1];
-    int64_t len = e - a;
-    uint8_t stackbuf[4096];
-    uint8_t* buf = stackbuf;
-    if (len + 8 > (int64_t)sizeof(stackbuf)) buf = new uint8_t[len + 8];
-    uint64_t t = tag;
-    __builtin_memcpy(buf, &t, 8);
-    __builtin_memcpy(buf + 8, b + a, len);
-    lo[i] = pw_xxh64_bytes(buf, len + 8, PW_SEED_LO);
-    hi[i] = pw_xxh64_bytes(buf, len + 8, PW_SEED_HI);
-    if (buf != stackbuf) delete[] buf;
+    const int64_t a = offsets[i], e = offsets[i + 1];
+    const PwHash128 h = pw_xxh64_tagged2(b, nbytes, a, e - a, tag);
+    lo[i] = h.lo;
+    hi[i] = h.hi;
   }
 }
 
@@ -375,32 +303,26 @@
   return (int)hipGetLastError();
 }
 
-__global__ void k_varlen_hash_se(const uint8_t* bytes, const int64_t* starts,
-                                 const int64_t* ends, uint64_t tag, int64_t n,
-                                 uint64_t* lo, uint64_t* hi) {
+__global__ __launch_bounds__(PW_BLOCK) void k_varlen_hash_se(
+    const uint8_t* __restrict__ bytes, int64_t nbytes,
+    const int64_t* __restrict__ starts, const int64_t* __restrict__ ends,
+    uint64_t tag, int64_t n, uint64_t* __restrict__ lo,
+    uint64_t* __restrict__ hi) {
   for (int64_t i = (int64_t)blockIdx.x * blockDim.x + threadIdx.x; i < n;
        i += (int64_t)gridDim.x * blockDim.x) {
-    int64_t a = starts[i], b = ends[i];
-    uint8_t buf[64];
-    int64_t len = b - a;
-    if (len <= 56) {
-      uint64_t t = tag;
-      __builtin_memcpy(buf, &t, 8);
-      for (int64_t k = 0; k < len; ++k) buf[8 + k] = bytes[a + k];
-      lo[i] = pw_xxh64_bytes(buf, 8 + len, PW_SEED_LO);
-      hi[i] = pw_xxh64_bytes(buf, 8 + len, PW_SEED_HI);
-    } else {
-      lo[i] = pw_xxh64_long(bytes + a, len, tag, PW_SEED_LO);
-      hi[i] = pw_xxh64_long(bytes + a, len, tag, PW_SEED_HI);
-    }
-  }
-}
-
-extern "C" int pw_varlen_hash_se(const void* bytes, const void* starts,
-                                 const void* ends, uint64_t tag, int64_t n,
-                                 void* lo, void* hi, void* stream) {
+    const int64_t a = starts[i], b = ends[i];
+    const PwHash128 h = pw_xxh64_tagged2(bytes, nbytes, a, b - a, tag);
+    lo[i] = h.lo;
+    hi[i] = h.hi;
+  }
+}
+
+extern "C" int pw_varlen_hash_se(const void* bytes, int64_t nbytes,
+                                 const void* starts, const void* ends,
+                                 uint64_t tag, int64_t n, void* lo, void* hi,
+                                 void* stream) {
   hipLaunchKernelGGL(k_varlen_hash_se, dim3(pw_grid(n)), dim3(PW_BLOCK), 0,
-                     (hipStream_t)stream, (const uint8_t*)bytes,
+                     (hipStream_t)stream, (const uint8_t*)bytes, nbytes,
                      (const int64_t*)starts, (const int64_t*)ends, tag, n,
                      (uint64_t*)lo, (uint64_t*)hi);
   return (int)hipGetLastError();
@@ -1726,77 +1648,152 @@
 }
 
 
+#define HT_SLOT_WORDS 4
+#define PW_HT_PROBE_Q 2
+#define HT_WORD_VAL 2
+
+extern "C" int pw_ht_slot_words() { return HT_SLOT_WORDS; }
+
+struct PwHtKey {
+  long long lo, hi;
+};
+
+static_assert(HT_SLOT_WORDS % 2 == 0, "16-byte key loads need even slots");
+
+struct PwHt {
+  long long* w;
+  __device__ __forceinline__ long long* slot(uint64_t s) const {
+    return w + s * HT_SLOT_WORDS;
+  }
+  __device__ __forceinline__ long long* val(uint64_t s) const {
+    return slot(s) + HT_WORD_VAL;
+  }
+  __device__ __forceinline__ PwHtKey key(uint64_t s) const {
+    const longlong2 v = *(const longlong2*)slot(s);
+    PwHtKey k;
+    k.lo = v.x, k.hi = v.y;
+    return k;
+  }
+  __device__ __forceinline__ void set_key(uint64_t s, long long lo,
+                                          long long hi) const {
+    longlong2 v;
+    v.x = lo, v.y = hi;
+    *(longlong2*)slot(s) = v;
+  }
+};
+
 __global__ void k_ht_build(const int64_t* __restrict__ klo,
                            const int64_t* __restrict__ khi,
                            const int64_t* __restrict__ vals, int64_t m,
-                           int64_t* tab_lo, int64_t* tab_hi,
-                           long long* tab_val, int64_t mask) {
+                           PwHt tab, int64_t mask) {
   int64_t i = (int64_t)blockIdx.x * blockDim.x + threadIdx.x;
   int64_t stride = (int64_t)gridDim.x * blockDim.x;
   for (; i < m; i += stride) {
     uint64_t slot = (uint64_t)klo[i] & (uint64_t)mask;
-    while (atomicCAS((unsigned long long*)&tab_val[slot],
+    while (atomicCAS((unsigned long long*)tab.val(slot),
                      (unsigned long long)(long long)-1,
                      (unsigned long long)(long long)(vals ? vals[i] : i)) !=
            (unsigned long long)(long long)-1)
       slot = (slot + 1) & (uint64_t)mask;
-    tab_lo[slot] = klo[i];
-    tab_hi[slot] = khi[i];
-  }
-}
-
-__global__ void k_ht_probe(const int64_t* __restrict__ qlo,
-                           const int64_t* __restrict__ qhi, int64_t nq,
-                           const int64_t* __restrict__ tab_lo,
-                           const int64_t* __restrict__ tab_hi,
-                           const long long* __restrict__ tab_val,
-                           int64_t mask, int64_t* out, bool* found) {
+    tab.set_key(slot, klo[i], khi[i]);
+  }
+}
+
+__device__ __forceinline__ long long pw_ht_find(const PwHt tab, uint64_t mask,
+                                                long long lo, long long hi,
+                                                int64_t max_probes) {
+  uint64_t slot = (uint64_t)lo & mask;
+  for (int64_t probes = 0; probes < max_probes; ++probes) {
+    const PwHtKey k = tab.key(slot);
+    const long long tv = *tab.val(slot);
+    if (tv < 0) return -1;
+    if (k.lo == lo && k.hi == hi) return tv;
+    slot = (slot + 1) & mask;
+  }
+  return -1;
+}
+
+__global__ __launch_bounds__(PW_BLOCK) void k_ht_probe(
+    const int64_t* __restrict__ qlo, const int64_t* __restrict__ qhi,
+    int64_t nq, const PwHt tab, int64_t mask, int64_t* __restrict__ out,
+    bool* __restrict__ found) {
   int64_t i = (int64_t)blockIdx.x * blockDim.x + threadIdx.x;
   int64_t stride = (int64_t)gridDim.x * blockDim.x;
-  for (; i < nq; i += stride) {
-    int64_t lo = qlo[i], hi = qhi[i];
-    uint64_t slot = (uint64_t)lo & (uint64_t)mask;
-    int64_t v = -1;
-    for (;;) {
-      long long tv = tab_val[slot];
-      if (tv == -1) break;
-      if (tab_lo[slot] == lo && tab_hi[slot] == hi) {
-        v = (int64_t)tv;
-        break;
-      }
-      slot = (slot + 1) & (uint64_t)mask;
-    }
-    out[i] = v;
-    found[i] = v != -1;
+  for (; i < nq; i += stride * PW_HT_PROBE_Q) {
+    long long lo[PW_HT_PROBE_Q], hi[PW_HT_PROBE_Q], v[PW_HT_PROBE_Q];
+    uint64_t slot[PW_HT_PROBE_Q];
+    bool live[PW_HT_PROBE_Q];
+    bool any = false;
+#pragma unroll
+    for (int q = 0; q < PW_HT_PROBE_Q; ++q) {
+      const int64_t j = i + q * stride;
+      live[q] = j < nq;
+      lo[q] = live[q] ? qlo[j] : 0;
+      hi[q] = live[q] ? qhi[j] : 0;
+      slot[q] = (uint64_t)lo[q] & (uint64_t)mask;
+      v[q] = -1;
+      any |= live[q];
+    }
+    for (int64_t probes = 0; any && probes <= mask; ++probes) {
+      PwHtKey k[PW_HT_PROBE_Q];
+      long long tv[PW_HT_PROBE_Q];
+#pragma unroll
+      for (int q = 0; q < PW_HT_PROBE_Q; ++q)
+        if (live[q]) {
+          k[q] = tab.key(slot[q]);
+          tv[q] = *tab.val(slot[q]);
+        }
+      any = false;
+#pragma unroll
+      for (int q = 0; q < PW_HT_PROBE_Q; ++q)
+        if (live[q]) {
+          if (tv[q] < 0) {
+            live[q] = false;
+          } else if (k[q].lo == lo[q] && k[q].hi == hi[q]) {
+            v[q] = tv[q];
+            live[q] = false;
+          } else {
+            slot[q] = (slot[q] + 1) & (uint64_t)mask;
+            any = true;
+          }
+        }
+    }
+#pragma unroll
+    for (int q = 0; q < PW_HT_PROBE_Q; ++q) {
+      const int64_t j = i + q * stride;
+      if (j < nq) {
+        out[j] = v[q];
+        found[j] = v[q] != -1;
+      }
+    }
   }
 }
 
 extern "C" int pw_ht_build(const void* klo, const void* khi, const void* vals,
-                           int64_t m, void* tab_lo, void* tab_hi,
-                           void* tab_val, int64_t nslots, void* stream) {
+                           int64_t m, void* tab, int64_t nslots,
+                           void* stream) {
   hipStream_t s = (hipStream_t)stream;
   int64_t nblocks = (m + PW_BLOCK - 1) / PW_BLOCK;
   if (nblocks > 4096) nblocks = 4096;
   if (nblocks < 1) nblocks = 1;
   hipLaunchKernelGGL(k_ht_build, dim3((uint32_t)nblocks), dim3(PW_BLOCK), 0, s,
                      (const int64_t*)klo, (const int64_t*)khi,
-                     (const int64_t*)vals, m, (int64_t*)tab_lo,
-                     (int64_t*)tab_hi, (long long*)tab_val, nslots - 1);
+                     (const int64_t*)vals, m, PwHt{(long long*)tab},
+                     nslots - 1);
   return (int)hipGetLastError();
 }
 
 extern "C" int pw_ht_probe(const void* qlo, const void* qhi, int64_t nq,
-                           const void* tab_lo, const void* tab_hi,
-                           const void* tab_val, int64_t nslots, void* out,
+                           const void* tab, int64_t nslots, void* out,
                            void* found, void* stream) {
   hipStream_t s = (hipStream_t)stream;
-  int64_t nblocks = (nq + PW_BLOCK - 1) / PW_BLOCK;
+  const int64_t per_block = (int64_t)PW_BLOCK * PW_HT_PROBE_Q;
+  int64_t nblocks = (nq + per_block - 1) / per_block;
   if (nblocks > 4096) nblocks = 4096;
   if (nblocks < 1) nblocks = 1;
   hipLaunchKernelGGL(k_ht_probe, dim3((uint32_t)nblocks), dim3(PW_BLOCK), 0, s,
                      (const int64_t*)qlo, (const int64_t*)qhi, nq,
-                     (const int64_t*)tab_lo, (const int64_t*)tab_hi,
-                     (const long long*)tab_val, nslots - 1, (int64_t*)out,
+                     PwHt{(long long*)tab}, nslots - 1, (int64_t*)out,
                      (bool*)found);
   return (int)hipGetLastError();
 }
@@ -1808,12 +1805,8 @@
 
 __global__ void k_ht_intern_claim(const int64_t* __restrict__ qlo,
                                   const int64_t* __restrict__ qhi, int64_t n,
-                                  const int64_t* tab_lo, const int64_t* tab_hi,
-                                  long long* tab_val, int64_t nslots,
-                                  const int64_t* __restrict__ front_lo,
-                                  const int64_t* __restrict__ front_hi,
-                                  const long long* __restrict__ front_val,
-                                  int64_t front_nslots,
+                                  const PwHt tab, int64_t nslots,
+                                  const PwHt front, int64_t front_nslots,
                                   int64_t* __restrict__ codes,
                                   uint8_t* __restrict__ pend, long long* err) {
   const uint64_t mask = (uint64_t)(nslots - 1);
@@ -1823,14 +1816,7 @@
   for (; i < n; i += stride) {
     const int64_t lo = qlo[i], hi = qhi[i];
     if (front_nslots) {
-      uint64_t fs = (uint64_t)lo & fmask;
-      long long fv = -1;
-      for (int64_t probes = 0; probes < front_nslots; ++probes) {
-        fv = front_val[fs];
-        if (fv < 0 || (front_lo[fs] == lo && front_hi[fs] == hi)) break;
-        fs = (fs + 1) & fmask;
-        fv = -1;
-      }
+      const long long fv = pw_ht_find(front, fmask, lo, hi, front_nslots);
       if (fv >= 0) {
         codes[i] = (int64_t)fv;
         pend[i] = 0;
@@ -1842,10 +1828,10 @@
     int64_t out = -1;
     uint8_t p = 0;
     int e = PW_HT_ERR_PROBE;
-    long long tv = tab_val[slot];
+    long long tv = *tab.val(slot);
     for (int64_t probes = 0; probes < nslots; ++probes) {
       if (tv == -1) {
-        tv = (long long)atomicCAS((unsigned long long*)&tab_val[slot],
+        tv = (long long)atomicCAS((unsigned long long*)tab.val(slot),
                                   (unsigned long long)(long long)-1,
                                   (unsigned long long)me);
         if (tv == -1) {
@@ -1854,7 +1840,8 @@
         }
       }
       if (tv >= 0) {
-        if (tab_lo[slot] == lo && tab_hi[slot] == hi) {
+        const PwHtKey k = tab.key(slot);
+        if (k.lo == lo && k.hi == hi) {
           out = (int64_t)tv, e = 0;
           break;
         }
@@ -1866,14 +1853,14 @@
         }
         if (qlo[r] == lo && qhi[r] == hi) {
           if (me > tv)
-            __hip_atomic_fetch_max(&tab_val[slot], me, __ATOMIC_RELAXED,
+            __hip_atomic_fetch_max(tab.val(slot), me, __ATOMIC_RELAXED,
                                    __HIP_MEMORY_SCOPE_AGENT);
           out = (int64_t)slot, p = 1, e = 0;
           break;
         }
       }
       slot = (slot + 1) & mask;
-      tv = tab_val[slot];
+      tv = *tab.val(slot);
     }
     if (e) atomicOr((unsigned long long*)err, (unsigned long long)e);
     codes[i] = out;
@@ -1883,7 +1870,7 @@
 
 __global__ void k_ht_intern_count(int64_t n, int64_t chunk,
                                   const int64_t* __restrict__ codes,
-                                  uint8_t* pend, const long long* tab_val,
+                                  uint8_t* pend, const PwHt tab,
                                   int64_t nslots, long long* block_counts,
                                   long long* err) {
   __shared__ int cnt;
@@ -1907,7 +1894,7 @@
         pend[i] = 0;
         continue;
       }
-      if (tab_val[slot] == -(long long)(i + 2)) {
+      if (*tab.val((uint64_t)slot) == -(long long)(i + 2)) {
         pend[i] = 2;
         ++local;
       }
@@ -1922,8 +1909,8 @@
     const int64_t* __restrict__ qlo, const int64_t* __restrict__ qhi,
     int64_t n, int64_t chunk, int64_t* codes, const uint8_t* __restrict__ pend,
     const long long* __restrict__ block_counts,
-    const long long* __restrict__ base_ptr, int64_t* tab_lo, int64_t* tab_hi,
-    long long* tab_val, int64_t* pool_lo, int64_t* pool_hi, int64_t pool_cap,
+    const long long* __restrict__ base_ptr, const PwHt tab, int64_t* pool_lo,
+    int64_t* pool_hi, int64_t pool_cap,
     int64_t* first_row, long long* n_new, long long* err) {
   const int lane = threadIdx.x & 63;
   const int wave = threadIdx.x >> 6;
@@ -1977,12 +1964,11 @@
                  (unsigned long long)PW_HT_ERR_CAPACITY);
       } else {
         const int64_t lo = qlo[i], hi = qhi[i];
-        tab_lo[slot] = lo;
-        tab_hi[slot] = hi;
+        tab.set_key((uint64_t)slot, lo, hi);
         pool_lo[code] = lo;
         pool_hi[code] = hi;
         first_row[k] = i;
-        tab_val[slot] = code;
+        *tab.val((uint64_t)slot) = code;
         codes[i] = code;
       }
       ++k;
@@ -1995,7 +1981,7 @@
 
 __global__ void k_ht_intern_resolve(int64_t n, int64_t chunk, int64_t* codes,
                                     const uint8_t* __restrict__ pend,
-                                    const long long* __restrict__ tab_val) {
+                                    const PwHt tab) {
   int64_t start = (int64_t)blockIdx.x * chunk;
   int64_t end = min(start + chunk, n);
   for (int64_t tile = start; tile < end; tile += (int64_t)blockDim.x * 16) {
@@ -2007,7 +1993,7 @@
     }
     for (int64_t i = g; i < min(g + 16, end); ++i) {
       if (pend[i] != 1) continue;
-      long long tv = tab_val[codes[i]];
+      long long tv = *tab.val((uint64_t)codes[i]);
       codes[i] = tv >= 0 ? (int64_t)tv : -1;
     }
   }
@@ -2019,9 +2005,7 @@
 }
 
 extern "C" int pw_ht_intern(const void* qlo, const void* qhi, int64_t n,
-                            void* tab_lo, void* tab_hi, void* tab_val,
-                            int64_t nslots, const void* front_lo,
-                            const void* front_hi, const void* front_val,
+                            void* tab, int64_t nslots, const void* front,
                             int64_t front_nslots, const void* base_ptr,
                             void* pool_lo, void* pool_hi, int64_t pool_cap,
                             void* codes, void* pend, void* first_row,
@@ -2034,28 +2018,26 @@
   int64_t cblocks = (n + PW_BLOCK - 1) / PW_BLOCK;
   if (cblocks > 4096) cblocks = 4096;
   int64_t chunk = pw_intern_chunk(n, nblocks);
+  const PwHt t{(long long*)tab};
+  const PwHt f{(long long*)const_cast<void*>(front)};
   hipLaunchKernelGGL(k_ht_intern_claim, dim3((uint32_t)cblocks),
                      dim3(PW_BLOCK), 0, s, (const int64_t*)qlo,
-                     (const int64_t*)qhi, n, (const int64_t*)tab_lo,
-                     (const int64_t*)tab_hi, (long long*)tab_val, nslots,
-                     (const int64_t*)front_lo, (const int64_t*)front_hi,
-                     (const long long*)front_val, front_nslots,
+                     (const int64_t*)qhi, n, t, nslots, f, front_nslots,
                      (int64_t*)codes, (uint8_t*)pend, (long long*)err);
   hipLaunchKernelGGL(k_ht_intern_count, dim3((uint32_t)nblocks),
                      dim3(PW_BLOCK), 0, s, n, chunk, (const int64_t*)codes,
-                     (uint8_t*)pend, (const long long*)tab_val, nslots,
-                     (long long*)block_counts, (long long*)err);
+                     (uint8_t*)pend, t, nslots, (long long*)block_counts,
+                     (long long*)err);
   hipLaunchKernelGGL(k_ht_intern_commit, dim3((uint32_t)nblocks),
                      dim3(PW_BLOCK), 0, s, (const int64_t*)qlo,
                      (const int64_t*)qhi, n, chunk, (int64_t*)codes,
                      (const uint8_t*)pend, (const long long*)block_counts,
-                     (const long long*)base_ptr, (int64_t*)tab_lo,
-                     (int64_t*)tab_hi, (long long*)tab_val, (int64_t*)pool_lo,
+                     (const long long*)base_ptr, t, (int64_t*)pool_lo,
                      (int64_t*)pool_hi, pool_cap, (int64_t*)first_row,
                      (long long*)n_new, (long long*)err);
   hipLaunchKernelGGL(k_ht_intern_resolve, dim3((uint32_t)nblocks),
                      dim3(PW_BLOCK), 0, s, n, chunk, (int64_t*)codes,
-                     (const uint8_t*)pend, (const long long*)tab_val);
+                     (const uint8_t*)pend, t);
   return (int)hipGetLastError();
 }
 
diff --git a/pathway_amd/ops/csrc/xxhash_common.h b/pathway_amd/ops/csrc/xxhash_common.h
--- a/pathway_amd/ops/csrc/xxhash_common.h
+++ b/pathway_amd/ops/csrc/xxhash_common.h
@@ -122,3 +122,135 @@
   }
   return pw_avalanche(h);
 }
+
+
+PW_HD uint32_t pw_tok_dword(uintptr_t q, uintptr_t tend, uintptr_t blo,
+                            uintptr_t bhi) {
+  if (q >= tend) return 0;
+  if (q >= blo && q + 4 <= bhi) {
+    uint32_t v;
+    __builtin_memcpy(&v, __builtin_assume_aligned((const void*)q, 4), 4);
+    return v;
+  }
+  uint32_t v = 0;
+  if (q + 0 >= blo && q + 0 < bhi) v |= (uint32_t)(*(const uint8_t*)(q + 0));
+  if (q + 1 >= blo && q + 1 < bhi) v |= (uint32_t)(*(const uint8_t*)(q + 1)) << 8;
+  if (q + 2 >= blo && q + 2 < bhi) v |= (uint32_t)(*(const uint8_t*)(q + 2)) << 16;
+  if (q + 3 >= blo && q + 3 < bhi) v |= (uint32_t)(*(const uint8_t*)(q + 3)) << 24;
+  return v;
+}
+
+struct PwTokReader {
+  uintptr_t q;
+  uintptr_t tend;
+  uintptr_t blo, bhi;
+  uint32_t carry;
+  int sh;
+};
+
+PW_HD void pw_tok_open(PwTokReader* r, const uint8_t* base, int64_t nbytes,
+                       int64_t a, int64_t len) {
+  const uintptr_t p = (uintptr_t)base + (uintptr_t)a;
+  r->blo = (uintptr_t)base;
+  r->bhi = (uintptr_t)base + (uintptr_t)nbytes;
+  r->tend = p + (uintptr_t)(len > 0 ? len : 0);
+  r->sh = (int)(p & 3) * 8;
+  r->q = p & ~(uintptr_t)3;
+  r->carry = pw_tok_dword(r->q, r->tend, r->blo, r->bhi);
+  r->q += 4;
+}
+
+PW_HD uint32_t pw_tok_next32(PwTokReader* r) {
+  const uint32_t d = pw_tok_dword(r->q, r->tend, r->blo, r->bhi);
+  const uint32_t v = (uint32_t)((((uint64_t)d << 32) | r->carry) >> r->sh);
+  r->carry = d;
+  r->q += 4;
+  return v;
+}
+
+PW_HD uint64_t pw_tok_next64(PwTokReader* r) {
+  const uint64_t lo = pw_tok_next32(r);
+  const uint64_t hi = pw_tok_next32(r);
+  return lo | (hi << 32);
+}
+
+struct PwHash128 {
+  uint64_t lo, hi;
+};
+
+PW_HD PwHash128 pw_xxh64_tagged2(const uint8_t* base, int64_t nbytes,
+                                 int64_t a, int64_t len, uint64_t tag) {
+  if (len < 0) len = 0;
+  PwTokReader r;
+  pw_tok_open(&r, base, nbytes, a, len);
+  int64_t rem = len;
+  uint64_t h0, h1;
+  if (len + 8 >= 32) {
+    uint64_t a1 = PW_SEED_LO + PW_P1 + PW_P2, b1 = PW_SEED_HI + PW_P1 + PW_P2;
+    uint64_t a2 = PW_SEED_LO + PW_P2, b2 = PW_SEED_HI + PW_P2;
+    uint64_t a3 = PW_SEED_LO, b3 = PW_SEED_HI;
+    uint64_t a4 = PW_SEED_LO - PW_P1, b4 = PW_SEED_HI - PW_P1;
+    uint64_t w = tag;
+    a1 = pw_round(a1, w), b1 = pw_round(b1, w);
+    w = pw_tok_next64(&r);
+    a2 = pw_round(a2, w), b2 = pw_round(b2, w);
+    w = pw_tok_next64(&r);
+    a3 = pw_round(a3, w), b3 = pw_round(b3, w);
+    w = pw_tok_next64(&r);
+    a4 = pw_round(a4, w), b4 = pw_round(b4, w);
+    rem -= 24;
+    while (rem >= 32) {
+      w = pw_tok_next64(&r);
+      a1 = pw_round(a1, w), b1 = pw_round(b1, w);
+      w = pw_tok_next64(&r);
+      a2 = pw_round(a2, w), b2 = pw_round(b2, w);
+      w = pw_tok_next64(&r);
+      a3 = pw_round(a3, w), b3 = pw_round(b3, w);
+      w = pw_tok_next64(&r);
+      a4 = pw_round(a4, w), b4 = pw_round(b4, w);
+      rem -= 32;
+    }
+    h0 = pw_rotl64(a1, 1) + pw_rotl64(a2, 7) + pw_rotl64(a3, 12) + pw_rotl64(a4, 18);
+    h0 = pw_merge_round(h0, a1);
+    h0 = pw_merge_round(h0, a2);
+    h0 = pw_merge_round(h0, a3);
+    h0 = pw_merge_round(h0, a4);
+    h1 = pw_rotl64(b1, 1) + pw_rotl64(b2, 7) + pw_rotl64(b3, 12) + pw_rotl64(b4, 18);
+    h1 = pw_merge_round(h1, b1);
+    h1 = pw_merge_round(h1, b2);
+    h1 = pw_merge_round(h1, b3);
+    h1 = pw_merge_round(h1, b4);
+    h0 += (uint64_t)(len + 8);
+    h1 += (uint64_t)(len + 8);
+  } else {
+    h0 = PW_SEED_LO + PW_P5 + (uint64_t)(len + 8);
+    h1 = PW_SEED_HI + PW_P5 + (uint64_t)(len + 8);
+    const uint64_t k = pw_round(0, tag);
+    h0 = pw_rotl64(h0 ^ k, 27) * PW_P1 + PW_P4;
+    h1 = pw_rotl64(h1 ^ k, 27) * PW_P1 + PW_P4;
+  }
+  while (rem >= 8) {
+    const uint64_t k = pw_round(0, pw_tok_next64(&r));
+    h0 = pw_rotl64(h0 ^ k, 27) * PW_P1 + PW_P4;
+    h1 = pw_rotl64(h1 ^ k, 27) * PW_P1 + PW_P4;
+    rem -= 8;
+  }
+  if (rem >= 4) {
+    const uint64_t k = (uint64_t)pw_tok_next32(&r) * PW_P1;
+    h0 = pw_rotl64(h0 ^ k, 23) * PW_P2 + PW_P3;
+    h1 = pw_rotl64(h1 ^ k, 23) * PW_P2 + PW_P3;
+    rem -= 4;
+  }
+  if (rem > 0) {
+    uint32_t t = pw_tok_next32(&r);
+    for (; rem > 0; --rem, t >>= 8) {
+      const uint64_t k = (uint64_t)(t & 0xFFu) * PW_P5;
+      h0 = pw_rotl64(h0 ^ k, 11) * PW_P1;
+      h1 = pw_rotl64(h1 ^ k, 11) * PW_P1;
+    }
+  }
+  PwHash128 out;
+  out.lo = pw_avalanche(h0);
+  out.hi = pw_avalanche(h1);
+  return out;
+}
diff --git a/profiles/ingest_kernels_bench.py b/profiles/ingest_kernels_bench.py
--- /dev/null
+++ b/profiles/ingest_kernels_bench.py
@@ -0,0 +1,82 @@
+
+from __future__ import annotations
+
+import json
+import statistics
+import time
+
+import torch
+
+from pathway_amd import ops
+from pathway_amd.internals.api import TAG_STR
+
+N = 4_000_000
+WW = 10
+CALLS = 30
+WARMUP = 5
+
+
+def timed(name: str, fn, **extra) -> None:
+    for _ in range(WARMUP):
+        fn()
+    ms = []
+    for _ in range(CALLS):
+        torch.cuda.synchronize()
+        t0 = time.perf_counter()
+        fn()
+        torch.cuda.synchronize()
+        ms.append((time.perf_counter() - t0) * 1e3)
+    print(json.dumps({
+        "op": name,
+        "median_ms": round(statistics.median(ms), 4),
+        "max_minus_min_ms": round(max(ms) - min(ms), 4),
+        "min_ms": round(min(ms), 4),
+        "calls": CALLS,
+        **extra,
+    }), flush=True)
+
+
+def main() -> None:
+    dev = torch.device("cuda:0")
+    g = torch.Generator(device=dev).manual_seed(1)
+
+    vocab = 50_000
+    words = torch.randint(97, 123, (vocab, WW), dtype=torch.uint8, device=dev,
+                          generator=g)
+    pick = torch.randint(0, vocab, (N,), device=dev, generator=g)
+    wire = torch.full((N, WW + 1), 10, dtype=torch.uint8, device=dev)
+    wire[:, :WW] = words[pick]
+    wire = wire.reshape(-1).contiguous()
+
+    timed("scan", lambda: ops.scan_positions_gpu(wire, 10), bytes=wire.numel())
+
+    nl = ops.scan_positions_gpu(wire, 10)
+    assert nl.numel() == N
+    starts = torch.cat([torch.zeros(1, dtype=torch.int64, device=dev),
+                        nl[:-1] + 1])
+    timed("hash", lambda: ops.varlen_hash_se_gpu(wire, starts, nl, TAG_STR),
+          tokens=N)
+
+    qlo, qhi = ops.varlen_hash_se_gpu(wire, starts, nl, TAG_STR)
+    voff = torch.arange(vocab + 1, dtype=torch.int64, device=dev) * WW
+    vlo, vhi = ops.varlen_hash_gpu(words.reshape(-1).contiguous(), voff, TAG_STR)
+    ht = ops.DeviceHashTable(vlo, vhi)
+    codes, found = ht.probe(qlo, qhi)
+    assert bool(found.all()) and torch.equal(vlo[codes], qlo)
+    timed("probe_50k", lambda: ht.probe(qlo, qhi), queries=N, keys=vocab,
+          nslots=ht.nslots)
+
+    big = 1_000_000
+    blo = torch.randint(-(1 << 62), 1 << 62, (big,), device=dev, generator=g)
+    bhi = torch.randint(-(1 << 62), 1 << 62, (big,), device=dev, generator=g)
+    ht_big = ops.DeviceHashTable(blo, bhi)
+    bq = torch.randint(0, big, (N,), device=dev, generator=g)
+    bqlo, bqhi = blo[bq], bhi[bq]
+    codes, found = ht_big.probe(bqlo, bqhi)
+    assert bool(found.all()) and torch.equal(blo[codes], bqlo)
+    timed("probe_1m", lambda: ht_big.probe(bqlo, bqhi), queries=N, keys=big,
+          nslots=ht_big.nslots)
+
+
+if __name__ == "__main__":
+    main()
```

After: 3.946 billion events/s, median of 6. 1.06x the previous value.
